# rvolden/C3POa

Measured on AMD Instinct MI355X. Metric: R2C2 reads->consensus/sec, higher is better.
Workload: dtype int32

## Files before the change

c3poa_amd/_lib.py:

```python
import ctypes as C
import os

import numpy as np

_HERE = os.path.dirname(os.path.abspath(__file__))
LIB_PATH = os.environ.get("C3POA_LIB", os.path.join(_HERE, "lib", "libc3poa_hip.so"))
MAX_PEAKS = 256

STAGE_CONK, STAGE_PEAKS, STAGE_POA, STAGE_POLISH, STAGES_ALL = 1, 2, 4, 8, 15
STAGE_QV = 16
QV_GLOBAL, QV_ANCHOR_START, QV_ANCHOR_END = 0, 1, 2
ST_OK, ST_NOT_ASSIGNED, ST_NO_PEAKS, ST_NO_CONSENSUS, ST_TOO_SHORT, ST_LIMIT = range(6)

EXPORTS = ["c3_default_config", "c3_version", "c3_device_count", "c3_warm_device", "c3_create", "c3_destroy", "c3_last_error", "c3_set_splints",
           "c3_batch_upload", "c3_batch_stage", "c3_batch_commit", "c3_batch_assign", "c3_batch_run", "c3_batch_sync", "c3_batch_results", "c3_batch_results_snapshot", "c3_batch_results_fetch", "c3_batch_timing",
           "c3_fetch_track", "c3_fetch_smoothed", "c3_fetch_raw_peaks", "c3_fetch_draft", "c3_fetch_msa2",
           "c3_call_peaks", "c3_poa_msa", "c3_pairwise_consensus", "c3_determine_consensus", "c3_zero_repeats", "c3_scan_splints",
           "c3_reader_open", "c3_reader_open_range", "c3_reader_close", "c3_reader_error", "c3_reader_names_only", "c3_reader_next", "c3_reader_next_set", "c3_reader_noqual", "c3_reader_reserved_bytes", "c3_reader_range_lost", "c3_write_group",
           "c3_scan_adapters", "c3_match_index", "c3_match_index_batch", "c3_demux_indexes", "c3_demux_host",
           "c3_assign_open", "c3_assign_close", "c3_assign_batch", "c3_assign_seen", "c3_write_splint_psl",
           "c3_host_alloc", "c3_host_free", "c3_writer_reset",
           "c3_batch_results_fetch_qv", "c3_batch_results_qv", "c3_batch_qv_timing", "c3_consensus_qv", "c3_consensus_qv_host",
           "c3_write_consensus_fastq",
           "c3_bgzf_create", "c3_bgzf_destroy", "c3_bgzf_bound", "c3_bgzf_compress", "c3_bgzf_compress_host",
           "c3_write_group_bgzf", "c3_write_consensus_fastq_bgzf",
           "c3_bgzf_scan", "c3_bgzf_decompress", "c3_bgzf_decompress_host", "c3_reader_open_inflate", "c3_reader_inflate_wait",
           "c3_fastq_parse", "c3_fastq_parse_host", "c3_reader_parse_on_device", "c3_reader_parse_stats", "c3_bam_parse", "c3_bam_parse_host",
           "c3_post_emit", "c3_post_emit_host", "c3_post_emit_timing",
           "c3_fasta_parse", "c3_fasta_parse_host", "c3_demux_emit", "c3_demux_emit_host", "c3_demux_emit_timing",
           "c3_emit_group", "c3_emit_group_host", "c3_batch_emit_snapshot", "c3_batch_emit_fetch", "c3_emit_timing_get", "c3_append_streams",
           "c3_fastx_strict_parse_host", "c3_post_emit_text", "c3_post_text_reset", "c3_post_text_timing_get",
           "c3_demux_emit_text", "c3_demux_emit_text_host", "c3_demux_text_reset", "c3_demux_text_timing_get",
           "c3_reader_stage_on_device", "c3_reader_device_group", "c3_reader_stage_stats"]


ZERO_MAX_CELLS = 16777216


class Config(C.Structure):
    _fields_ = ([("device", C.c_int), ("conk_match", C.c_int), ("conk_mismatch", C.c_int), ("conk_penalty", C.c_int),
                 ("sg_iters", C.c_int), ("sg_window", C.c_int), ("sg_order", C.c_int), ("mdistcutoff", C.c_int),
                 ("poa_match", C.c_int), ("poa_mismatch", C.c_int), ("poa_o1", C.c_int), ("poa_e1", C.c_int),
                 ("poa_o2", C.c_int), ("poa_e2", C.c_int), ("poa_band_b", C.c_int), ("poa_band_f", C.c_double),
                 ("pol_match", C.c_int), ("pol_mismatch", C.c_int), ("pol_gap", C.c_int), ("pol_window", C.c_int),
                 ("pol_q", C.c_int), ("dang_band", C.c_int), ("slots_poa", C.c_int), ("slots_win", C.c_int), ("zero", C.c_int),
                 ("zero_max_cells", C.c_int64)])


class ReadResult(C.Structure):
    _fields_ = [("status", C.c_int32), ("n_peaks", C.c_int32), ("n_sub", C.c_int32), ("has_front", C.c_int32),
                ("has_tail", C.c_int32), ("front_end", C.c_int32), ("tail_beg", C.c_int32), ("cons_len", C.c_int32),
                ("draft_len", C.c_int32), ("n_win", C.c_int32), ("peaks", C.c_int32 * MAX_PEAKS),
                ("sub_beg", C.c_int32 * MAX_PEAKS), ("sub_end", C.c_int32 * MAX_PEAKS)]


RESULT_DTYPE = np.dtype([("status", "<i4"), ("n_peaks", "<i4"), ("n_sub", "<i4"), ("has_front", "<i4"),
                         ("has_tail", "<i4"), ("front_end", "<i4"), ("tail_beg", "<i4"), ("cons_len", "<i4"),
                         ("draft_len", "<i4"), ("n_win", "<i4"), ("peaks", "<i4", (MAX_PEAKS,)),
                         ("sub_beg", "<i4", (MAX_PEAKS,)), ("sub_end", "<i4", (MAX_PEAKS,))])
assert RESULT_DTYPE.itemsize == C.sizeof(ReadResult)


class Timing(C.Structure):
    _fields_ = [(n, C.c_float) for n in ("ms_pack", "ms_conk", "ms_peaks", "ms_poa", "ms_prep", "ms_window",
                                         "ms_stitch", "ms_total")] + \
               [(n, C.c_int64) for n in ("n_reads", "n_bases", "n_windows", "cells_conk", "cells_poa", "cells_polish", "n_poa_redo")] + \
               [(n, C.c_float) for n in ("ms_wall", "ms_host_worklist", "ms_alloc", "ms_host_gap")] + \
               [(n, C.c_int64) for n in ("cells_polish_computed", "n_band_layers", "n_band_fallback", "n_band_mismatch", "n_win_redo", "n_poa_redo16")]


def _fields_dict(t):
    return {f[0]: getattr(t, f[0]) for f in t._fields_}


class _Info(C.Structure):

    def as_dict(self):
        return {k: int(getattr(self, k)) for k, _t in self._fields_}


class QvTiming(C.Structure):
    _fields_ = [("ms_qv", C.c_float)] + [(n, C.c_int64) for n in ("n_reads", "n_pieces", "n_skipped", "band_cells", "edge_hits")]


class FastaInfo(_Info):
    _fields_ = [(k, C.c_int64) for k in ("n_records", "consumed", "name_bytes", "base_bytes")] + [("departed", C.c_int32)]


class DemuxInfo(_Info):
    _fields_ = [(k, C.c_int64) for k in ("n_records", "n_kept", "consumed", "out_bytes")] + [("departed", C.c_int32)]


class DemuxTiming(C.Structure):
    _fields_ = [(n, C.c_float) for n in ("ms_parse", "ms_demux", "ms_emit", "ms_call")] + \
               [(n, C.c_int64) for n in ("n_records", "n_kept", "in_bytes", "out_bytes")]


class DemuxSetsStruct(C.Structure):
    _fields_ = [(k + f, t) for k in "ab" for f, t in (("_n", C.c_int), ("_cat", C.c_void_p), ("_off", C.c_void_p), ("_names", C.c_void_p), ("_name_off", C.c_void_p))]


class DemuxTextInfo(_Info):
    _fields_ = [(k, C.c_int64) for k in ("n_records", "n_kept", "consumed", "text_bytes", "out_bytes")] + \
               [(k, C.c_int32) for k in ("departed", "kind", "n_streams")]


class DemuxTextTiming(C.Structure):
    _fields_ = [(n, C.c_float) for n in ("ms_inflate", "ms_parse", "ms_demux", "ms_split", "ms_emit", "ms_bgzf", "ms_call")] + \
               [(n, C.c_int64) for n in ("n_records", "n_kept", "in_bytes", "text_bytes", "out_bytes")] + \
               [(n, C.c_int32) for n in ("n_streams", "n_waits")]


class FastqInfo(_Info):
    _fields_ = [(k, C.c_int64) for k in ("n_records", "n_kept", "n_short", "consumed", "name_bytes", "base_bytes")] + [("departed", C.c_int32)]


class BamInfo(_Info):
    _fields_ = [(k, C.c_int64) for k in ("n_records", "n_kept", "n_short", "consumed", "name_bytes", "base_bytes", "header_bytes", "bad_at")] + \
               [("departed", C.c_int32), ("reason", C.c_int32)]


class FastxInfo(_Info):
    _fields_ = [(k, C.c_int64) for k in ("n_records", "consumed", "name_bytes", "base_bytes")] + [("departed", C.c_int32)]


class PostTextInfo(_Info):
    _fields_ = [(k, C.c_int64) for k in ("n_records", "n_kept", "consumed", "text_bytes", "out_bytes")] + [("departed", C.c_int32)]


class PostTextTiming(C.Structure):
    _fields_ = [(n, C.c_float) for n in ("ms_inflate", "ms_parse", "ms_gather", "ms_adapter", "ms_post", "ms_bgzf", "ms_call")] + \
               [(n, C.c_int64) for n in ("n_records", "n_kept", "in_bytes", "text_bytes", "out_bytes")]


class PostArgs(C.Structure):
    _fields_ = [("n", C.c_int32), ("names", C.c_void_p), ("name_off", C.c_void_p), ("seqs", C.c_void_p), ("quals", C.c_void_p),
                ("off", C.c_void_p), ("table", C.c_void_p), ("n_ad", C.c_int32), ("ad_len", C.c_void_p), ("ad_class", C.c_void_p),
                ("class5", C.c_int32), ("ad_names", C.c_void_p), ("ad_name_off", C.c_void_p), ("has_index", C.c_int32),
                ("n_idx", C.c_int32), ("idx_cat", C.c_void_p), ("idx_off", C.c_void_p), ("idx_dest", C.c_void_p),
                ("n_dest", C.c_int32), ("undirectional", C.c_int32), ("trim", C.c_int32), ("barcoded", C.c_int32)]


class PostTiming(C.Structure):
    _fields_ = [(k, C.c_float) for k in ("ms_classify", "ms_scan", "ms_emit", "ms_call")] + \
               [(k, C.c_int64) for k in ("n_reads", "n_kept", "in_bytes", "out_bytes")]


class EmitTiming(C.Structure):
    _fields_ = [(k, C.c_float) for k in ("ms_len", "ms_scan", "ms_write", "ms_bgzf", "ms_call")] + \
               [(k, C.c_int64) for k in ("n_reads", "n_records", "in_bytes", "out_bytes")]


class HostBatchStruct(C.Structure):
    _fields_ = [("n", C.c_int32), ("n_short", C.c_int64), ("names", C.c_void_p), ("name_off", C.c_void_p),
                ("seqs", C.c_void_p), ("quals", C.c_void_p), ("off", C.c_void_p)]


class DeviceBatchStruct(C.Structure):
    _fields_ = [("d_seqs", C.c_void_p), ("d_quals", C.c_void_p), ("device", C.c_int32), ("bytes", C.c_int64)]


_lib = None


def load():
    global _lib
    if _lib is not None:
        return _lib
    if not os.path.exists(LIB_PATH):
        raise ImportError("c3poa_amd: %s is missing -- run `python -c 'import __graft_entry__ as g; g.build()'` "
                          "(there is no CPU fallback)" % LIB_PATH)
    lib = C.CDLL(LIB_PATH)
    vp, ip, cp, i64p = C.c_void_p, C.POINTER(C.c_int), C.c_char_p, C.c_void_p
    lib.c3_default_config.argtypes = [C.POINTER(Config)]
    lib.c3_version.restype = C.c_char_p
    lib.c3_create.argtypes = [C.POINTER(Config), C.POINTER(vp)]
    lib.c3_destroy.argtypes = [vp]
    lib.c3_destroy.restype = None
    lib.c3_last_error.argtypes = [vp]
    lib.c3_last_error.restype = C.c_char_p
    lib.c3_set_splints.argtypes = [vp, C.c_int, cp, i64p]
    lib.c3_batch_upload.argtypes = [vp, C.c_int, vp, vp, i64p, vp, vp]
    lib.c3_batch_stage.argtypes = [vp, C.c_int, vp, vp, i64p, vp, vp]
    lib.c3_batch_commit.argtypes = [vp]
    lib.c3_batch_assign.argtypes = [vp, vp, vp]
    lib.c3_batch_run.argtypes = [vp, C.c_int]
    lib.c3_batch_sync.argtypes = [vp]
    lib.c3_batch_results.argtypes = [vp, vp, vp, C.c_int64, i64p]
    lib.c3_batch_results_snapshot.argtypes = [vp]
    lib.c3_batch_results_fetch.argtypes = [vp, vp, vp, C.c_int64, i64p]
    lib.c3_batch_timing.argtypes = [vp, C.POINTER(Timing)]
    lib.c3_fetch_track.argtypes = [vp, C.c_int, vp, C.c_int64]
    lib.c3_fetch_smoothed.argtypes = [vp, C.c_int, vp, C.c_int64]
    lib.c3_fetch_raw_peaks.argtypes = [vp, C.c_int, vp, C.c_int]
    lib.c3_fetch_draft.argtypes = [vp, C.c_int, vp, C.c_int]
    lib.c3_fetch_msa2.argtypes = [vp, C.c_int, vp, vp, C.c_int]
    lib.c3_call_peaks.argtypes = [vp, vp, C.c_int, C.c_int, vp, C.c_int, vp]
    lib.c3_poa_msa.argtypes = [vp, C.c_int, C.POINTER(cp), ip, vp, C.c_int, ip, vp, C.c_int64, ip]
    lib.c3_zero_repeats.argtypes = [vp, cp, cp, C.c_int, cp, cp, C.c_int, C.c_int, vp, C.c_int, ip]
    lib.c3_scan_splints.argtypes = [vp, vp, vp, vp]
    lib.c3_pairwise_consensus.argtypes = [vp, cp, cp, C.c_int, cp, C.c_int, cp, cp, C.c_int, cp, vp, C.c_int, ip]
    lib.c3_scan_adapters.argtypes = [vp, vp]
    lib.c3_match_index.argtypes = [cp, C.c_int, C.c_int, cp, vp]
    lib.c3_match_index_batch.argtypes = [vp, C.c_int, vp, vp, C.c_int, cp, vp, vp]
    lib.c3_demux_indexes.argtypes = [vp, C.c_int, vp, C.c_int, cp, vp, C.c_int, cp, vp, vp, vp]
    lib.c3_demux_host.argtypes = [C.c_int, vp, C.c_int, cp, vp, C.c_int, cp, vp, vp, vp]
    lib.c3_assign_open.argtypes = [cp, C.c_int, C.POINTER(cp), C.POINTER(vp)]
    lib.c3_assign_close.argtypes = [vp]
    lib.c3_assign_close.restype = None
    lib.c3_assign_batch.argtypes = [vp, C.POINTER(HostBatchStruct), vp, vp]
    lib.c3_assign_seen.argtypes = [vp, vp, vp]
    lib.c3_write_splint_psl.argtypes = [C.POINTER(HostBatchStruct), vp, vp, vp, C.c_int, C.POINTER(cp), vp, C.c_int, cp, vp]
    lib.c3_host_alloc.argtypes = [C.c_int64, C.POINTER(vp)]
    lib.c3_host_free.argtypes = [vp]
    lib.c3_host_free.restype = None
    lib.c3_writer_reset.restype = None
    lib.c3_reader_open.argtypes = [cp, C.c_int, C.POINTER(vp)]
    lib.c3_reader_open_range.argtypes = [cp, C.c_int, C.c_int64, C.c_int64, C.POINTER(vp)]
    lib.c3_reader_close.argtypes = [vp]
    lib.c3_reader_close.restype = None
    lib.c3_reader_error.argtypes = [vp]
# ... 1464 lines not shown
```

c3poa_amd/csrc/c3_args.h:

```cpp
#pragma once
#include "c3_dev.h"
#include <cstddef>

struct C3Counters {
  int queue;
  int peaks_queue;
  unsigned long long cells;
  unsigned long long cells_computed;
  unsigned long long zero_cells;
  int poa_ovf;
  int poa_ovf16;
  int n_windows;
  int win_ovf;
  int win_queue2;
  int band_layers, band_fallback;
  int band_mismatch;
  struct { int window, layer, R, q, band_row, full_row, next_row; } verify;
  unsigned long long phases[16];
};
static_assert(offsetof(C3Counters, cells) % 8 == 0 && offsetof(C3Counters, cells_computed) % 8 == 0 &&
              offsetof(C3Counters, zero_cells) % 8 == 0 && offsetof(C3Counters, phases) % 8 == 0, "u64 counters must be 8-byte aligned");

struct ConkArgs {
  C3Batch b; const uint8_t* sp_codes; const int* sp_len; int32_t* track; C3Info* info; C3Counters* cnt;
  int match, mismatch, penalty;
  int n_spl; int32_t* scan;
};
struct PeaksArgs {
  C3Batch b; const int32_t* track; C3Info* info; double* bufA; double* bufB; int32_t* cand; uint8_t* cstate;
  int32_t* raw_peaks; int32_t* n_raw; const int* sp_len; double coef[64]; int64_t maxL; int window, iters, min_dist;
  C3Counters* cnt;
};
struct PoaArgs {
  C3Batch b; C3Info* info; C3Params p; C3Counters* cnt; const int* work; int n_work;
  int* ibase; int* ebase; char* cellsb; uint8_t* bbase; long long* score;
  int Ncap, K, Pcap, cells_cap;
  uint8_t* draft; int32_t* tpos; uint8_t* msa_dbg; const int64_t* msa_off; int* msa_len;
  int rb_span;
  int no2col;
  uint4* desc; int* jump;
  int* pbase;
  int* overflow;
  int* overflow16;
};
#define C3_POA_NI 19
__host__ __device__ inline int c3_poa_far_shift(bool w32) { return w32 ? 0 : 2; }
struct PoaLayout { size_t ints, edges, cells, bases, score, desc, jump, path, total; };
__host__ __device__ inline PoaLayout c3_poa_layout(size_t Ncap, size_t K, int cells_cap, int far_shift, size_t Pcap) {
  PoaLayout l;
  l.ints = sizeof(int) * C3_POA_NI * Ncap; l.edges = sizeof(int) * 3 * Ncap * K;
  l.cells = 2 * (size_t)cells_cap + 16 * (size_t)(cells_cap >> far_shift);
  l.bases = 5 * Ncap; l.score = sizeof(long long) * Ncap; l.desc = sizeof(uint4) * 2 * Ncap;
  l.jump = sizeof(int) * C3_JUMP_LEVELS * Ncap; l.path = sizeof(int) * Pcap;
  l.total = l.ints + l.edges + l.cells + l.bases + l.score + l.desc + l.jump + l.path;
  return l;
}

struct WLayer { int qbeg, len, begin, end; };
struct WinRec { int rid, w, n_layers, blen, tgs, out_len, polished, pad_; };
struct PrepArgs {
  C3Batch b; C3Info* info; C3Params p; C3Counters* cnt; const int* work; int n_work;
  const uint8_t* draft; int32_t* tpos; int wcap; uint8_t* eD; int64_t ecap; int* lw_first; int* lw_last; int NLcap, NWcap;
  WinRec* wrec; WLayer* wlay; int* win_base;
  int sub_shift;
  int rows_old;
};
struct WinArgs {
  C3Batch b; C3Params p; C3Counters* cnt; int n_win; const WinRec* wrec_in; WinRec* wrec; const WLayer* wlay; int NLcap;
  const uint8_t* draft;
  uint8_t* base; int* ibase; int* ebase; long long* score;
  int32_t* H; uint16_t* D; uint4* rdesc; int Ncap, K; long long hcap; uint8_t* wout; int wout_cap;
  int Lcap;
  int band_mode;
  const int* wlist; int* ovf_list;
  int no_chain;
};
#define W_INTS 19
struct WinLayout { size_t ints, edges, bases, score, H, D, desc, total; };
__host__ __device__ inline WinLayout c3_win_layout(size_t Ncap, size_t K, size_t hcap) {
  WinLayout l;
  l.ints = sizeof(int) * W_INTS * Ncap; l.edges = sizeof(int) * 4 * Ncap * K; l.bases = 2 * Ncap; l.score = sizeof(long long) * Ncap;
  l.H = sizeof(int32_t) * hcap; l.D = hcap; l.desc = sizeof(uint4) * (Ncap + 1);
  l.total = l.ints + l.edges + l.bases + l.score + l.H + l.D + l.desc;
  return l;
}
struct StitchArgs {
  C3Batch b; C3Info* info; const int* work; int n_work; const WinRec* wrec; const int* win_base; const uint8_t* wout; int wout_cap; char* cons;
  const uint8_t* zflag;
};
struct AdapterArgs {
  C3Batch b; C3Params p; C3Counters* cnt;
  const uint8_t* ad_codes; const int* ad_len; int n_ad;
  uint8_t* D; long long dcap;
  int32_t* out;
};

struct ZeroArgs {
  C3Batch b; C3Info* info; C3Params p; C3Counters* cnt; const int* work; int n_work;
  uint8_t* D; long long dcap;
  int4* zinfo; uint8_t* zflag;
  const uint8_t* draft; char* cons;
  uint8_t* S; long long scap; int zk;
};

struct ZlLayout { long long ck, dir, car, total; };
__host__ __device__ inline ZlLayout c3_zl_layout(long long n0, long long n1, long long K) {
  ZlLayout l;
  l.ck = 0;
  l.dir = (n1 + K - 1) / K * (n0 + 1) * 8;
  l.car = (l.dir + (n1 < K ? n1 : K) * (n0 + 1) + 15) & ~15LL;
  l.total = (l.car + n1 * 12 + 255) & ~255LL;
  return l;
}
struct QvArgs {
  int n_reads; const C3Info* info; const uint32_t* pk; const int64_t* woff; const uint8_t* qual; const int64_t* off;
  const char* cons; char* qv;
  int sa_np, sa_n; const int64_t* sa_woff; const int64_t* sa_off; const int32_t* sa_mode;
  uint32_t* dirs; long long dir_words;
  int* gS; uint8_t* gcodes; long long gcap;
  int lds_n;
  unsigned long long* cnt;
};
```

c3poa_amd/csrc/c3_handle.hip:

```cpp
#include "c3_host.h"
#include "c3_bgzf.h"

thread_local double c3h::g_alloc_ms = 0.0;

__device__ __forceinline__ uint32_t pack_code(uint32_t b) {
  const uint32_t u = b & 0xDFu;
  const uint32_t c = (u >> 1) & 3u;
  const bool ok = (u == 'A') | (u == 'C') | (u == 'G') | (u == 'T') | (u == 'U');
  return ok ? (c ^ (c >> 1)) : 0u;
}
__global__ __launch_bounds__(256) void k_pack(const uint8_t* ascii, const int64_t* off, const int64_t* woff, int n, uint32_t* pk) {
  const int lane = threadIdx.x & 63;
  const int wave = (blockIdx.x * blockDim.x + threadIdx.x) >> 6, n_waves = (gridDim.x * blockDim.x) >> 6;
  for (int r = wave; r < n; r += n_waves) {
    const int64_t L = off[r + 1] - off[r];
    const int64_t nw = woff[r + 1] - woff[r];
    const uint8_t* s = ascii + off[r];
    uint32_t* dst = pk + woff[r];
    for (int64_t w = lane; w < nw; w += 64) {
      uint32_t x = 0;
      if (w * 16 + 16 <= L) {
        uint32_t v[4];
        __builtin_memcpy(v, s + w * 16, 16);
#pragma unroll
// ... 20 lines not shown
__device__ __forceinline__ long long cons_len_of(const C3Info* p) { return p->status == C3_ST_OK ? (long long)p->cons_len : 0; }
__global__ __launch_bounds__(256) void k_coff_sums(const C3Info* info, int n, long long* part) {
  __shared__ long long sh[256];
  const int i = blockIdx.x * 256 + threadIdx.x;
  sh[threadIdx.x] = i < n ? cons_len_of(info + i) : 0;
  __syncthreads();
  for (int d = 128; d > 0; d >>= 1) { if ((int)threadIdx.x < d) sh[threadIdx.x] += sh[threadIdx.x + d]; __syncthreads(); }
  if (threadIdx.x == 0) part[blockIdx.x] = sh[0];
}
__global__ __launch_bounds__(1024) void k_coff_scan(long long* part, int nb, int64_t* coff, int n) {
  __shared__ long long sh[1024];
  long long carry = 0;
  for (int b0 = 0; b0 < nb; b0 += 1024) {
    const int b = b0 + threadIdx.x;
    const long long v = b < nb ? part[b] : 0;
    sh[threadIdx.x] = v;
    __syncthreads();
    for (int d = 1; d < 1024; d <<= 1) { long long t = (int)threadIdx.x >= d ? sh[threadIdx.x - d] : 0; __syncthreads(); sh[threadIdx.x] += t; __syncthreads(); }
    if (b < nb) part[b] = carry + sh[threadIdx.x] - v;
    carry += sh[1023];
    __syncthreads();
  }
  if (threadIdx.x == 0) { coff[0] = 0; coff[n] = carry; }
}
__global__ __launch_bounds__(256) void k_coff_final(const C3Info* info, int n, const long long* part, int64_t* coff) {
  __shared__ long long sh[256];
  const int i = blockIdx.x * 256 + threadIdx.x;
  sh[threadIdx.x] = i < n ? cons_len_of(info + i) : 0;
  __syncthreads();
  for (int d = 1; d < 256; d <<= 1) { long long t = (int)threadIdx.x >= d ? sh[threadIdx.x - d] : 0; __syncthreads(); sh[threadIdx.x] += t; __syncthreads(); }
  if (i < n) coff[i + 1] = part[blockIdx.x] + sh[threadIdx.x];
}
__global__ void k_init_info(C3Info* info, int n) {
  int i = blockIdx.x * blockDim.x + threadIdx.x;
  if (i < n) { C3Info* p = &info[i]; p->status = C3_ST_OK; p->n_peaks = 0; p->n_sub = 0; p->has_front = p->has_tail = 0;
               p->front_end = p->tail_beg = 0; p->cons_len = 0; p->draft_len = 0; p->n_win = 0; }
}

extern "C" void c3_default_config(c3_config* c) {
  memset(c, 0, sizeof(*c));
  c->device = 0;
  c->conk_match = 5; c->conk_mismatch = -4; c->conk_penalty = 20;
  c->sg_iters = 3; c->sg_window = 41; c->sg_order = 2; c->mdistcutoff = 500;
  c->poa_match = 5; c->poa_mismatch = 4; c->poa_o1 = 4; c->poa_e1 = 2; c->poa_o2 = 24; c->poa_e2 = 1;
  c->poa_band_b = 10; c->poa_band_f = 0.01;
  c->pol_match = 3; c->pol_mismatch = -5; c->pol_gap = -4; c->pol_window = 500; c->pol_q = 5; c->dang_band = 128;
  c->slots_poa = 0; c->slots_win = 0; c->zero = 1; c->zero_max_cells = 16 << 20;
}
extern "C" const char* c3_version(void) { return "c3poa_amd 0.1 (gfx950)"; }
extern "C" int c3_device_count(void) { int n = 0; if (hipGetDeviceCount(&n) != hipSuccess) { (void)hipGetLastError(); return 0; } return n; }

extern "C" int c3_warm_device(int device) {
  int n = 0;
  if (hipGetDeviceCount(&n) != hipSuccess || device < 0 || device >= n) { (void)hipGetLastError(); return C3_E_NO_DEVICE; }
  if (hipSetDevice(device) != hipSuccess || hipFree(nullptr) != hipSuccess) { (void)hipGetLastError(); return C3_E_HIP; }
  return C3_E_OK;
}

static thread_local std::string g_create_err;
extern "C" const char* c3_last_error(const c3_handle* h) { return h ? h->err.c_str() : g_create_err.c_str(); }
void c3_set_host_error(const char* msg) { g_create_err = msg; }

static int check_poa_scoring(const c3_config* cfg) {
  const struct { const char* name; int v, lo, hi; } f[6] = {
    {"poa_match", cfg->poa_match, 1, 64}, {"poa_mismatch", cfg->poa_mismatch, 0, 64},
    {"poa_o1", cfg->poa_o1, 0, 64}, {"poa_e1", cfg->poa_e1, 0, 16}, {"poa_o2", cfg->poa_o2, 0, 64}, {"poa_e2", cfg->poa_e2, 0, 16}};
  for (const auto& x : f) {
    if (x.v < x.lo || x.v > x.hi) {
      char buf[160];
      snprintf(buf, sizeof buf, "%s = %d: must be %d..%d (the 16-bit cells of k_poa and their guard are exact in that range only)", x.name, x.v, x.lo, x.hi);
      return host_fail(C3_E_ARG, buf);
    }
  }
  return C3_E_OK;
}

static int check_pol_scoring(const c3_config* cfg) {
  const struct { const char* name; int v; } f[3] = {{"pol_match", cfg->pol_match}, {"pol_mismatch", cfg->pol_mismatch}, {"pol_gap", cfg->pol_gap}};
  for (const auto& x : f) {
    if (x.v < -C3_POL_MAX || x.v > C3_POL_MAX) {
      char buf[160];
      snprintf(buf, sizeof buf, "%s = %d: must be %d..%d (the 32-bit cells of the polish rows and their sentinels are exact in that range only)", x.name, x.v, -C3_POL_MAX, C3_POL_MAX);
      return host_fail(C3_E_ARG, buf);
    }
  }
  if (cfg->pol_match <= 2 * cfg->pol_gap) {
    char buf[200];
    snprintf(buf, sizeof buf, "pol_match = %d: must be above 2 * pol_gap = %d (a match that scores no more than two gaps makes every layer a chain of new nodes, beyond the window graph's capacity)",
             cfg->pol_match, 2 * cfg->pol_gap);
    return host_fail(C3_E_ARG, buf);
  }
  return C3_E_OK;
}

static int check_pol_window(const c3_config* cfg) {
  char buf[200];
  if (cfg->pol_window < 1 || cfg->pol_window > C3_POL_WINDOW_MAX) {
    snprintf(buf, sizeof buf, "pol_window = %d: must be %d..%d (a window graph of 3 * pol_window + 40 nodes per layer has to stay below the 65535 node ids k_window's consensus holds)",
             cfg->pol_window, 1, C3_POL_WINDOW_MAX);
    return host_fail(C3_E_ARG, buf);
  }
  if (cfg->dang_band < 0) {
    snprintf(buf, sizeof buf, "dang_band = %d: must be %d..%d (the half width of the extension band; 0 is the diagonal alone)", cfg->dang_band, 0, 255);
    return host_fail(C3_E_ARG, buf);
  }
  return C3_E_OK;
}

extern "C" int c3_create(const c3_config* cfg, c3_handle** out) {
  if (!cfg || !out) return C3_E_ARG;
  *out = nullptr;
  if (int rc = check_poa_scoring(cfg)) return rc;
  if (int rc = check_pol_scoring(cfg)) return rc;
  if (int rc = check_pol_window(cfg)) return rc;
  int ndev = 0;
  hipError_t e = hipGetDeviceCount(&ndev);
  if (e != hipSuccess || ndev <= 0) return host_fail(C3_E_NO_DEVICE, "no HIP device: the c3poa HIP backend has no CPU fallback");
  if (cfg->device < 0 || cfg->device >= ndev) return host_fail(C3_E_ARG, "bad device ordinal");
  if (cfg->conk_match < -127 || cfg->conk_match > 127 || cfg->conk_mismatch < -127 || cfg->conk_mismatch > 127) {
    return host_fail(C3_E_ARG, "conk_match / conk_mismatch must fit a signed byte");
  }
  if (cfg->dang_band > 255) return host_fail(C3_E_LIMIT, "dang_band must be at most 255 (k_prep holds 512 band offsets per wave)");
  if (cfg->sg_order != 2 && cfg->sg_order != 3) return host_fail(C3_E_ARG, "sg_order must be 2 or 3");
  if (cfg->sg_window < 5 || cfg->sg_window > 127 || !(cfg->sg_window & 1)) return host_fail(C3_E_ARG, "sg_window must be odd, 5..127");
  if (cfg->zero_max_cells < 1 || cfg->zero_max_cells > INT32_MAX) return host_fail(C3_E_ARG, "zero_max_cells must be 1..2147483647");
  c3_handle* h = new c3_handle();
  h->cfg = *cfg;
  hipDeviceProp_t prop;
  e = hipSetDevice(cfg->device);
  if (e == hipSuccess) {
    (void)hipSetDeviceFlags(hipDeviceScheduleBlockingSync); (void)hipGetLastError();
    e = hipGetDeviceProperties(&prop, cfg->device);
  }
  if (e == hipSuccess) e = hipStreamCreate(&h->stream);
  if (e == hipSuccess) e = hipStreamCreate(&h->stream_up);
  if (e == hipSuccess) e = hipStreamCreate(&h->stream_dn);
  if (e == hipSuccess) e = hipEventCreateWithFlags(&h->ev_dn, hipEventDisableTiming);
  if (e == hipSuccess) e = hipHostMalloc((void**)&h->h_tot, 64, hipHostMallocDefault);
  for (int i = 0; i < 2 && e == hipSuccess; ++i) e = hipEventCreate(&h->ev_up[i]);
  for (int i = 0; i < EV_N && e == hipSuccess; ++i) e = hipEventCreate(&h->ev[i]);
  if (e != hipSuccess) { c3_destroy(h); return host_fail(C3_E_HIP, hipGetErrorString(e)); }
  h->n_cus = prop.multiProcessorCount > 0 ? prop.multiProcessorCount : 256;
  h->mem_total = prop.totalGlobalMem;
  memset(&h->tm, 0, sizeof(h->tm));
  *out = h;
  return C3_E_OK;
}

extern "C" void c3_destroy(c3_handle* h) {
  if (!h) return;
  (void)hipSetDevice(h->cfg.device);
  for (hipStream_t s : {h->stream, h->stream_up, h->stream_dn}) if (s) (void)hipStreamSynchronize(s);
  for (hipStream_t s : {h->stream, h->stream_up, h->stream_dn}) if (s) (void)hipStreamDestroy(s);
  for (hipEvent_t ev : {h->ev_dn, h->ev_up[0], h->ev_up[1], h->ev_qv[0], h->ev_qv[1]}) if (ev) (void)hipEventDestroy(ev);
  for (hipEvent_t ev : h->ev) if (ev) (void)hipEventDestroy(ev);
  for (hipEvent_t ev : h->ev_post) if (ev) (void)hipEventDestroy(ev);
  for (hipEvent_t ev : h->ev_fa) if (ev) (void)hipEventDestroy(ev);
  for (c3h::EmitBufs* eb : {&h->emit_sa, &h->emit_snap}) for (hipEvent_t ev : eb->ev) if (ev) (void)hipEventDestroy(ev);
  if (h->ev_emit_dn) (void)hipEventDestroy(h->ev_emit_dn);
  if (h->h_fa_hdr) (void)hipHostFree(h->h_fa_hdr);
  c3h::post_text_free(h);
  c3h::demux_text_free(h);
  if (h->h_tot) (void)hipHostFree(h->h_tot);
  delete h;
}

extern "C" int c3_set_splints(c3_handle* h, int n, const char* cat, const int64_t* off) {
  if (!h || n <= 0 || !cat || !off) return C3_E_ARG;
  HIPCHK(hipSetDevice(h->cfg.device));
  std::vector<uint8_t> codes((size_t)n * 2 * C3_SPLINT_MAX, 0);
  std::vector<int> sp_len((size_t)n, 0); int max_spl = 0;
  for (int i = 0; i < n; ++i) {
    int S = (int)(off[i + 1] - off[i]);
    if (S <= 0 || S > C3_SPLINT_MAX) return c3_fail(h, C3_E_LIMIT, "splint length must be 1..512");
    if ((long long)std::max({h->cfg.conk_match, h->cfg.conk_mismatch, 0}) * S > 32000 || h->cfg.conk_penalty < 0 || h->cfg.conk_penalty > 32000)
      return c3_fail(h, C3_E_LIMIT, "max(conk_match, conk_mismatch) * splint length and conk_penalty must stay within 32000 (16-bit score cells in k_conk)");
    sp_len[(size_t)i] = S; max_spl = std::max(max_spl, S);
    for (int k = 0; k < S; ++k) {
      int c = code_of(cat[off[i] + k]);
      codes[((size_t)i * 2 + 0) * C3_SPLINT_MAX + k] = (uint8_t)c;
      codes[((size_t)i * 2 + 1) * C3_SPLINT_MAX + (S - 1 - k)] = (uint8_t)(3 - c);
    }
  }
  HIPCHK(h->d_sp_codes.put(codes.data(), codes.size(), h->stream));
  HIPCHK(h->d_sp_len.put(sp_len.data(), sizeof(int) * n, h->stream));
  HIPCHK(hipStreamSynchronize(h->stream));
  h->sp_len.swap(sp_len); h->max_spl = max_spl; h->n_spl = n;
  return C3_E_OK;
}

extern "C" int c3_batch_stage(c3_handle* h, int n, const char* seqs, const char* quals, const int64_t* off,
                              const int16_t* splint_id, const char* strand) {
  if (!h || n <= 0 || !seqs || !quals || !off || !strand) return C3_E_ARG;
  if (h->n_spl <= 0) return c3_fail(h, C3_E_STATE, "c3_set_splints must be called first");
  if (h->st.pending) return c3_fail(h, C3_E_STATE, "a staged batch is waiting for c3_batch_commit");
  HIPCHK(hipSetDevice(h->cfg.device));
  if (off[0] != 0) return c3_fail(h, C3_E_ARG, "off[0] must be 0");
  c3_handle::Staged& t = h->st;
  t.n = n; t.total = off[n] - off[0]; t.off.assign(off, off + n + 1); t.woff.assign(n + 1, 0); t.maxL = 0;
  t.sid.assign((size_t)n, 0); t.strand.assign(strand, (size_t)n);
  for (int i = 0; i < n; ++i) {
    int64_t L = off[i + 1] - off[i];
    if (L < 0 || L > (1 << 30)) return c3_fail(h, C3_E_ARG, "bad read length");
    t.maxL = std::max(t.maxL, L);
    t.woff[i + 1] = t.woff[i] + (L + 15) / 16 + 2;
    if (splint_id) { if (splint_id[i] < 0 || splint_id[i] >= h->n_spl) return c3_fail(h, C3_E_ARG, "splint_id out of range"); t.sid[i] = splint_id[i]; }
  }
  t.words = t.woff[n];
  const size_t T = (size_t)t.total;
  HIPCHK(t.d_ascii.ensure(T + 16)); HIPCHK(t.d_pk.ensure(sizeof(uint32_t) * (size_t)t.words + 64));
  HIPCHK(t.d_qual.ensure(T + 16)); HIPCHK(t.d_off.ensure(sizeof(int64_t) * (n + 1))); HIPCHK(t.d_woff.ensure(sizeof(int64_t) * (n + 1)));
  HIPCHK(t.d_strand.ensure(n)); HIPCHK(t.d_sid.ensure(sizeof(int16_t) * n));
  hipStream_t su = h->stream_up;
  HIPCHK(hipEventRecord(h->ev_up[0], su));
  HIPCHK(hipMemcpyAsync(t.d_ascii.p, seqs, T, hipMemcpyHostToDevice, su));
  HIPCHK(hipMemcpyAsync(t.d_qual.p, quals, T, hipMemcpyHostToDevice, su));
  HIPCHK(hipMemcpyAsync(t.d_off.p, t.off.data(), sizeof(int64_t) * (n + 1), hipMemcpyHostToDevice, su));
  HIPCHK(hipMemcpyAsync(t.d_woff.p, t.woff.data(), sizeof(int64_t) * (n + 1), hipMemcpyHostToDevice, su));
  HIPCHK(hipMemcpyAsync(t.d_strand.p, t.strand.data(), n, hipMemcpyHostToDevice, su));
  HIPCHK(hipMemcpyAsync(t.d_sid.p, t.sid.data(), sizeof(int16_t) * n, hipMemcpyHostToDevice, su));
  c3k_launch_pack(t.d_ascii.as<uint8_t>(), t.d_off.as<int64_t>(), t.d_woff.as<int64_t>(), n, t.d_pk.as<uint32_t>(), std::min((n + 3) / 4, h->n_cus * 32), su);
  HIPCHK(hipEventRecord(h->ev_up[1], su));
  HIPCHK(hipGetLastError());
  t.pending = true;
  return C3_E_OK;
}

extern "C" int c3_batch_commit(c3_handle* h) {
  if (!h) return C3_E_ARG;
  if (!h->st.pending) return c3_fail(h, C3_E_STATE, "no staged batch");
  HIPCHK(hipSetDevice(h->cfg.device));
  HIPCHK(hipStreamSynchronize(h->stream));
  HIPCHK(hipStreamSynchronize(h->stream_up));
  c3_handle::Staged& t = h->st;
  std::swap(h->d_ascii, t.d_ascii); std::swap(h->d_pk, t.d_pk); std::swap(h->d_woff, t.d_woff); std::swap(h->d_qual, t.d_qual);
  std::swap(h->d_off, t.d_off); std::swap(h->d_strand, t.d_strand); std::swap(h->d_sid, t.d_sid);
  h->off.swap(t.off); h->woff.swap(t.woff);
  h->n = t.n; h->total = t.total; h->words = t.words; h->maxL = t.maxL;
  t.pending = false;
  const int n = h->n;
  HIPCHK(h->d_info.ensure(sizeof(C3Info) * (size_t)n));
  HIPCHK(h->d_counter.ensure(sizeof(C3Counters)));
  HIPCHK(hipMemsetAsync(h->d_info.p, 0, sizeof(C3Info) * (size_t)n, h->stream));
  hipLaunchKernelGGL(k_init_info, dim3((n + 255) / 256), dim3(256), 0, h->stream, h->d_info.as<C3Info>(), n);
  HIPCHK(hipStreamSynchronize(h->stream));
  HIPCHK(hipGetLastError());
  float ms = 0; HIPCHK(hipEventElapsedTime(&ms, h->ev_up[0], h->ev_up[1]));
  memset(&h->tm, 0, sizeof(h->tm)); h->tm.ms_pack = ms; h->tm.n_reads = n; h->tm.n_bases = h->total;
  h->stages_done = 0; h->injected = false; h->n_windows = 0; h->res_prefix = 0;
  return C3_E_OK;
}

extern "C" int c3_batch_assign(c3_handle* h, const int16_t* splint_id, const char* strand) {
  if (!h || h->n <= 0 || !splint_id || !strand) return C3_E_ARG;
  HIPCHK(hipSetDevice(h->cfg.device));
  std::vector<int16_t> sid((size_t)h->n);
  for (int i = 0; i < h->n; ++i) {
    const bool on = strand[i] == '+' || strand[i] == '-';
    if (on && (splint_id[i] < 0 || splint_id[i] >= h->n_spl)) return c3_fail(h, C3_E_ARG, "splint_id out of range");
    sid[(size_t)i] = on ? splint_id[i] : (int16_t)0;
  }
  HIPCHK(hipMemcpyAsync(h->d_strand.p, strand, (size_t)h->n, hipMemcpyHostToDevice, h->stream));
  HIPCHK(hipMemcpyAsync(h->d_sid.p, sid.data(), sizeof(int16_t) * (size_t)h->n, hipMemcpyHostToDevice, h->stream));
  hipLaunchKernelGGL(k_init_info, dim3((h->n + 255) / 256), dim3(256), 0, h->stream, h->d_info.as<C3Info>(), h->n);
  HIPCHK(hipStreamSynchronize(h->stream));
  HIPCHK(hipGetLastError());
  h->stages_done = 0;
  return C3_E_OK;
}

extern "C" int c3_batch_upload(c3_handle* h, int n, const char* seqs, const char* quals, const int64_t* off,
                               const int16_t* splint_id, const char* strand) {
  if (h && h->st.pending) { (void)hipStreamSynchronize(h->stream_up); h->st.pending = false; }
  int rc = c3_batch_stage(h, n, seqs, quals, off, splint_id, strand);
  if (rc != C3_E_OK) return rc;
  return c3_batch_commit(h);
}

extern "C" int c3_batch_qv_timing(c3_handle* h, c3_qv_timing* t) {
  if (!h || !t) return C3_E_ARG;
  *t = h->qtm;
  return C3_E_OK;
}

extern "C" int c3_batch_sync(c3_handle* h) {
  if (!h) return C3_E_ARG;
  HIPCHK(hipSetDevice(h->cfg.device));
  HIPCHK(hipStreamSynchronize(h->stream));
  return C3_E_OK;
}

extern "C" int c3_batch_results_snapshot(c3_handle* h) {
  if (!h || h->n <= 0) return C3_E_ARG;
  if (h->snap_pending.load(std::memory_order_acquire)) return c3_fail(h, C3_E_STATE, "c3_batch_results_snapshot: the previous snapshot has not been fetched");
  HIPCHK(hipSetDevice(h->cfg.device));
  const int n = h->n;
  DBuf& d_coff = h->d_gather_off; DBuf& d_out = h->d_gather;
  const int nb = (n + 255) / 256;
  HIPCHK(d_coff.ensure(sizeof(int64_t) * (size_t)(n + 1))); HIPCHK(h->d_coff_part.ensure(sizeof(long long) * (size_t)nb));
  hipLaunchKernelGGL(k_coff_sums, dim3(nb), dim3(256), 0, h->stream, h->d_info.as<C3Info>(), n, h->d_coff_part.as<long long>());
  hipLaunchKernelGGL(k_coff_scan, dim3(1), dim3(1024), 0, h->stream, h->d_coff_part.as<long long>(), nb, d_coff.as<int64_t>(), n);
  hipLaunchKernelGGL(k_coff_final, dim3(nb), dim3(256), 0, h->stream, h->d_info.as<C3Info>(), n, h->d_coff_part.as<long long>(), d_coff.as<int64_t>());
  long long tot = 0;
  const bool have_cons = (h->stages_done & C3_STAGE_POLISH) != 0;
  if (have_cons) {
    HIPCHK(hipMemcpyAsync(h->h_tot, d_coff.as<int64_t>() + n, sizeof(long long), hipMemcpyDeviceToHost, h->stream));
    HIPCHK(hipStreamSynchronize(h->stream));
// ... 269 lines not shown
```

c3poa_amd/csrc/c3_host.h:

```cpp
#pragma once
#include "c3_dev.h"
#include "c3_args.h"
#include "c3_launch.h"
#include "c3_checks.h"
#include "c3_emit.h"
#include "c3_post.h"
#include "c3_fastx.h"
#include "c3_dsplit.h"
#include "c3_bgzf.h"
#include <algorithm>
#include <atomic>
#include <chrono>
#include <cstddef>
#include <cstdio>
#include <cstdlib>
#include <cstring>
#include <functional>
#include <string>
#include <vector>

struct c3_handle;
namespace c3h {
extern thread_local double g_alloc_ms;
int qv_scratch(c3_handle* h, long long max_m, long long max_n, int n_items, QvArgs& a, int* grid);
int fetch_msa_rows(c3_handle* h, int read, int nrows, char* out, int64_t cap, int* msa_len);
struct EmitBufs;
int emit_run(c3_handle* h, EmitArgs& p, EmitBufs& eb, hipStream_t s, std::vector<int64_t>& so, int64_t cap);
int post_sizes(c3_handle* h, const c3_post_args* a, PostArgs& p, std::vector<int64_t>& so);
int post_write(c3_handle* h, PostArgs& p, int64_t need);
int adapters_device(c3_handle* h, const C3Batch& b, int64_t max_len, int32_t* d_out);
int bgzf_inflate_to_device(c3_bgzf* z, const char* src, int64_t n, int64_t nm, uint8_t* d_dst, int64_t* out_len);
namespace fa { enum { FA_TEXT, FA_CNT, FA_NL, FA_LSE, FA_LDST, FA_BSUM, FA_HDR, FA_OFF, FA_NOFF, FA_RECL, FA_HASH, FA_NAMES, FA_SEQS, FA_KREC, FA_ROFF,
                      FA_OUT, FA_ANAMES, FA_ANO, FA_BNAMES, FA_BNO, FA_N }; }
int fasta_parse_resident(c3_handle* h, const uint8_t* d_text, int64_t n, int at_eof, int kept, FaArgs* a);
int fasta_gather_resident(c3_handle* h, FaArgs* a);
int demux_sets_device(c3_handle* h, const c3_demux_sets* st, const uint8_t* tab, int K, int64_t nk, FaArgs* a);
struct ZStage;
struct ZStatus { hipError_t e = hipSuccess; enum { OK, MEMBER_SIZE, BEYOND_BOUND } bad = OK; const char* what = ""; int waits = 0; };
typedef std::function<hipError_t(char* d_zin, int64_t c0, int64_t cn)> ZStageIn;
ZStatus bgzf_chunks(ZStage& z, hipStream_t s, int64_t len, const ZStageIn& stage_in, char* arena, int64_t cap, int64_t* out, bool wait_after_copy_out);
struct TextFront;
struct TextLoad { int nxt = 0, kind = 0, waits = 0; int64_t total = 0; float ms_inflate = 0; };
void text_free(TextFront& t);
void text_reset(TextFront& t);
int text_load(c3_handle* h, TextFront& t, const char* src, int64_t n, bool in_z, bool keep_q, const char* who, const char* keep_flag,
              hipEvent_t* ev, int n_ev, TextLoad* ld);
int text_tables(c3_handle* h, TextFront& t, const TextLoad& ld, int at_eof, FxArgs& f, int* waits, hipEvent_t ev_begin = nullptr, hipEvent_t ev_records = nullptr);
int text_gather(c3_handle* h, TextFront& t, FxArgs& f, bool keep_q, hipEvent_t ev_begin = nullptr);
void text_commit(TextFront& t, const TextLoad& ld, int64_t consumed, int at_eof);
int bgzf_stream_device(c3_handle* h, ZStage& z, const char* d_src, int64_t len, char* arena, int64_t cap, int64_t* out, int* waits = nullptr);
void post_text_free(c3_handle* h);
void demux_text_free(c3_handle* h);
}

#define BGZF_CHUNK_BLOCKS 2048

static inline double dbg_now_ms() { using namespace std::chrono; return duration<double, std::milli>(steady_clock::now().time_since_epoch()).count(); }
#define DBG(...) do { if (getenv("C3_DEBUG")) { fprintf(stderr, "[c3 %.3f] ", dbg_now_ms()); fprintf(stderr, __VA_ARGS__); fflush(stderr); } } while (0)

struct DBuf {
  void* p = nullptr; size_t cap = 0;
  DBuf() = default;
  DBuf(DBuf&& o) noexcept : p(o.p), cap(o.cap) { o.p = nullptr; o.cap = 0; }
  DBuf& operator=(DBuf&& o) noexcept { std::swap(p, o.p); std::swap(cap, o.cap); return *this; }
  DBuf(const DBuf&) = delete;
  DBuf& operator=(const DBuf&) = delete;
  ~DBuf() { if (p) (void)hipFree(p); }
  hipError_t ensure(size_t bytes) {
    if (bytes <= cap) return hipSuccess;
    const double t0 = dbg_now_ms();
    if (p) { hipError_t e = hipFree(p); p = nullptr; cap = 0; if (e != hipSuccess) return e; }
    size_t want = bytes + bytes / 8 + 256;
    hipError_t e = hipMalloc(&p, want);
    if (e == hipSuccess) cap = want;
    if (e == hipSuccess && getenv("C3_DEBUG_POISON")) e = hipMemset(p, 0xA5, want);
    c3h::g_alloc_ms += dbg_now_ms() - t0;
    return e;
  }
  hipError_t put(const void* src, size_t bytes, hipStream_t s, size_t slack = 0) {
    const hipError_t e = ensure(bytes + slack);
    return e != hipSuccess ? e : hipMemcpyAsync(p, src, bytes, hipMemcpyHostToDevice, s);
  }
  template <class T> T* as() const { return (T*)p; }
};

struct c3h::EmitBufs { DBuf work, offs, arena; hipEvent_t ev[5] = {}; };

struct c3h::ZStage {
  DBuf zin, zslots, zsizes, zpacked; int* h_sizes = nullptr;
  ~ZStage() { if (h_sizes) (void)hipHostFree(h_sizes); }
  hipError_t pin() { return h_sizes ? hipSuccess : hipHostMalloc((void**)&h_sizes, BGZF_CHUNK_BLOCKS * sizeof(int), hipHostMallocDefault); }
  hipError_t reserve(int64_t cn) {
    cn = std::min(cn, (int64_t)BGZF_CHUNK_BLOCKS * BGZF_BLOCK);
    const size_t nb = (size_t)((cn + BGZF_BLOCK - 1) / BGZF_BLOCK);
    hipError_t e = pin();
    if (e == hipSuccess) e = zin.ensure((size_t)cn + 256);
    if (e == hipSuccess) e = zslots.ensure(nb * BGZF_SLOT);
    if (e == hipSuccess) e = zsizes.ensure(nb * sizeof(int));
    if (e == hipSuccess) e = zpacked.ensure(nb * BGZF_MAX_MEMBER);
    return e;
  }
};
struct c3h::TextFront {
  DBuf text[2]; int cur = 0, kind = 0; int64_t text_n = 0, tail_from = 0;
  DBuf cnt, nl, slen, nlen, bsum, hdr, lhdr, off, name_off, woff, src, hash, names, seqs, quals;
  ZStage zs;
  C3FxHdr* h_hdr = nullptr; C3FqHdr* h_lhdr = nullptr; c3_bgzf* z = nullptr;
};
struct PostText : c3h::TextFront {
  DBuf pk, table;
  hipEvent_t ev[8] = {};
  c3_post_text_timing tm = {};
};
struct DemuxText : c3h::TextFront {
  DBuf krec, kb, nkept, key, rank, base, soff, out;
  int64_t* h_soff = nullptr;
  hipEvent_t ev[6] = {};
  c3_demux_text_timing tm = {};
};

struct Summary { int status, n_sub, max_sub, sum_sub, max_dang, front, tail, n_peaks; };
enum { EV_N = 10 };
struct c3_handle {
  c3_config cfg; std::string err; hipStream_t stream = nullptr; int n_cus = 256; size_t mem_total = 0;
  hipStream_t stream_up = nullptr; hipEvent_t ev_up[2] = {nullptr, nullptr};
  hipStream_t stream_dn = nullptr; hipEvent_t ev_dn = nullptr; long long* h_tot = nullptr;
  std::atomic<bool> snap_pending{false}; int snap_n = 0, snap_kp = 0; long long snap_tot = 0; bool snap_cons = false;
  DBuf d_info_snap, d_coff_part;
  struct Staged { DBuf d_ascii, d_pk, d_woff, d_qual, d_off, d_strand, d_sid; std::vector<int64_t> off, woff; std::vector<int16_t> sid; std::string strand;
                  int n = 0; int64_t total = 0, words = 0, maxL = 0; bool pending = false; } st;
  hipEvent_t ev[EV_N] = {};
  int n_spl = 0, max_spl = 0; std::vector<int> sp_len; DBuf d_sp_codes, d_sp_len;
  int n = 0; int64_t total = 0, words = 0, maxL = 0; std::vector<int64_t> off, woff;
  DBuf d_ascii, d_pk, d_woff, d_qual, d_off, d_strand, d_sid, d_info, d_track, d_draft, d_tpos, d_cons, d_counter, d_gather, d_gather_off;
  DBuf d_raw, d_nraw, d_sum, d_work, d_bufA, d_bufB, d_cand, d_cst, d_msa, d_msa_off, d_msa_len;
  DBuf s_poa_i, s_poa_nk, s_poa_cells, s_poa_b, s_poa_sc, s_poa_desc, s_poa_jump, s_poa_path, d_overflow;
  int n_poa_redo = 0;
  int n_poa_redo16 = 0;
  DBuf s_eD, s_lw, d_wrec, d_wlay, d_wbase, d_wout;
  DBuf s_win_i, s_win_nk, s_win_h, s_win_d, s_win_b, s_win_sc, s_win_desc, s_win_h2, s_win_d2, d_wovf;
  DBuf s_zero_d, d_zinfo, d_zflag, d_zwork; std::vector<int> zwork;
  DBuf s_zero_l;
  DBuf d_dmx_heads, d_dmx_meta, d_dmx_out;
  DBuf d_qv, s_qv_dirs, s_qv_g, d_qv_cnt, d_gather_qv;
  hipEvent_t ev_qv[2] = {nullptr, nullptr}; c3_qv_timing qtm = {}; bool snap_qv = false;
  DBuf d_post[16]; hipEvent_t ev_post[5] = {}; c3_post_timing ptm = {};
  PostText pt;
  DemuxText dx; std::vector<uint32_t> dmx_meta_host;
  DBuf d_fa[20]; hipEvent_t ev_fa[10] = {}; c3_demux_timing dtm = {}; struct C3FaHdr* h_fa_hdr = nullptr;
  DBuf d_emit[10]; c3h::EmitBufs emit_sa; c3_emit_timing etm = {};
  c3h::EmitBufs emit_snap; DBuf d_emit_names, d_emit_noff; c3h::ZStage emit_zs;
  hipEvent_t ev_emit_dn = nullptr;
  std::atomic<bool> emit_pending{false}; int emit_S = 0, emit_flags = 0; std::vector<int64_t> emit_so; c3_emit_timing emit_tm = {};
  std::vector<Summary> sum; std::vector<int> work;
  int res_prefix = 0;
  int peaks_grid = 0; bool debug_msa = false; bool injected = false;
  int n_windows = 0;
  c3_timing tm;
  unsigned long long phase_poa[16] = {0}, phase_win[16] = {0};
  int stages_done = 0;
};

static inline int c3_hip_fail(c3_handle* h, hipError_t e, const char* what, const char* file, int line) {
  char buf[512];
  const char* base = strrchr(file, '/');
  snprintf(buf, sizeof buf, "HIP error %d (%s) at %s:%d: %s", (int)e, hipGetErrorString(e), base ? base + 1 : file, line, what);
  if (h) h->err = buf;
  return C3_E_HIP;
}
static inline int c3_fail(c3_handle* h, int code, const char* msg) { if (h) h->err = msg; return code; }
#define HIPCHK(x) do { hipError_t e_ = (x); if (e_ != hipSuccess) return c3_hip_fail(h, e_, #x, __FILE__, __LINE__); } while (0)
static inline int host_fail(int code, const char* msg) { c3_set_host_error(msg); return code; }
static inline int bgzf_fail(hipError_t e, const char* what) {
  char buf[256];
  snprintf(buf, sizeof buf, "HIP error %d (%s): %s", (int)e, hipGetErrorString(e), what);
  return host_fail(C3_E_HIP, buf);
}
#define ZCHK(x, what) do { hipError_t e_ = (x); if (e_ != hipSuccess) return bgzf_fail(e_, what); } while (0)

template <class T> struct Override {
  T& ref; const T saved;
  Override(T& r, T v) : ref(r), saved(r) { r = v; }
  ~Override() { ref = saved; }
  Override(const Override&) = delete;
};

static inline C3Counters* dev_cnt(c3_handle* h) { return h->d_counter.as<C3Counters>(); }
template <class T> static inline hipError_t zero_cnt(c3_handle* h, T* field) { return hipMemsetAsync(field, 0, sizeof(T), h->stream); }
static inline hipError_t read_counters(c3_handle* h, C3Counters* c) {
  hipError_t e = hipMemcpyAsync(c, h->d_counter.p, sizeof(*c), hipMemcpyDeviceToHost, h->stream);
  return e != hipSuccess ? e : hipStreamSynchronize(h->stream);
}

static inline int code_of(char c) {
  switch (c) { case 'C': case 'c': return 1; case 'G': case 'g': return 2; case 'T': case 't': case 'U': case 'u': return 3; default: return 0; }
}

static inline C3Batch dev_batch(c3_handle* h) {
  C3Batch b; b.n = h->n; b.pk = h->d_pk.as<uint32_t>(); b.woff = h->d_woff.as<int64_t>(); b.qual = h->d_qual.as<uint8_t>();
  b.off = h->d_off.as<int64_t>(); b.strand = h->d_strand.as<uint8_t>(); b.splint_id = h->d_sid.as<int16_t>();
  return b;
}
static inline C3Params dev_params(const c3_config& c) {
  C3Params p;
  p.conk_match = c.conk_match; p.conk_mismatch = c.conk_mismatch; p.conk_penalty = c.conk_penalty;
  p.sg_iters = c.sg_iters; p.sg_window = c.sg_window; p.sg_order = c.sg_order; p.mdist = c.mdistcutoff;
  p.poa_match = c.poa_match; p.poa_mismatch = c.poa_mismatch; p.o1 = c.poa_o1; p.e1 = c.poa_e1; p.o2 = c.poa_o2; p.e2 = c.poa_e2;
  p.band_b = c.poa_band_b; p.band_f = c.poa_band_f;
  p.pol_match = c.pol_match; p.pol_mismatch = c.pol_mismatch; p.pol_gap = c.pol_gap; p.pol_window = c.pol_window; p.pol_q = c.pol_q;
  p.dang_band = c.dang_band;
  p.zero = c.zero; p.zr_match = 2; p.zr_mismatch = 4; p.zr_gapo = 4; p.zr_gape = 2; p.zr_min_score = 80; p.zr_max_cells = (int)c.zero_max_cells;
  return p;
}

struct c3_bgzf {
  int device = 0; hipStream_t stream = nullptr;
  c3h::ZStage zs;
  C3BgzfMember* h_mem = nullptr; int2* h_res = nullptr;
  DBuf d_mem, d_res, d_out;
  struct FqSlot {
    DBuf text, names, seqs, quals, off, name_off, src;
    int64_t text_n = 0, n_rec = 0;
    int64_t* h_off = nullptr; int64_t* h_name_off = nullptr; size_t h_cap = 0;
  } fq[2];
  DBuf d_cnt, d_nl, d_slen, d_nlen, d_bsum, d_hdr;
  C3FqHdr* h_hdr = nullptr;
  DBuf d_tiles, d_rpos, d_reason, d_rsrc, d_bhdr;
  C3BamHdr* h_bhdr = nullptr;
  hipStream_t copy_stream = nullptr;
  struct DevSet { DBuf seqs, quals; };
  std::vector<DevSet> dsets;
};
```

c3poa_amd/csrc/c3_launch.h:

```cpp
#pragma once
#include <hip/hip_runtime.h>
#include <stddef.h>
#include <stdint.h>

struct ConkArgs; struct AdapterArgs; struct PostArgs; struct PeaksArgs; struct PoaArgs; struct PrepArgs; struct WinArgs; struct StitchArgs;
struct ZeroArgs; struct QvArgs; struct C3BgzfMember; struct C3FqHdr; struct C3BamHdr; struct C3BamTile; struct FaArgs; struct EmitArgs; struct FxArgs; struct DsArgs;

extern "C" {
void c3k_launch_conk(const ConkArgs*, int, int, int, hipStream_t);
void c3k_launch_adapter(const AdapterArgs*, int, hipStream_t);
void c3k_launch_match_index(const char*, const int*, int, int, const char*, const long long*, int*, hipStream_t);
void c3k_launch_pairwise(const uint8_t*, int, const uint8_t*, int, const uint8_t*, int, uint8_t*, uint8_t*, int*, hipStream_t);
void c3k_launch_poa(const PoaArgs*, int, int, int, hipStream_t);
void c3k_launch_post_classify(const PostArgs*, hipStream_t);
void c3k_launch_post_scan(const PostArgs*, hipStream_t);
void c3k_launch_post_emit(const PostArgs*, hipStream_t);
void c3k_launch_demux(const uint8_t*, int, const uint8_t*, int, int, int, int32_t*, uint8_t*, hipStream_t);
size_t c3k_demux_lds(int, int);
void c3k_launch_peaks(const PeaksArgs*, int, hipStream_t);
int c3k_peaks_blocks_per_cu(void);
void c3k_launch_prep(const PrepArgs*, int, hipStream_t);
void c3k_launch_window(const WinArgs*, int, hipStream_t);
void c3k_launch_stitch(const StitchArgs*, int, hipStream_t);
void c3k_launch_zero(const ZeroArgs*, int, hipStream_t);
void c3k_launch_zero_long(const ZeroArgs*, int, hipStream_t);
void c3k_launch_zero_finish(const ZeroArgs*, int, hipStream_t);
void c3k_launch_qv(const QvArgs*, int, hipStream_t);
int c3k_qv_lds_max(void);
void c3k_launch_bgzf(const uint8_t*, long long, int, uint8_t*, int*, uint8_t*, hipStream_t);
void c3k_launch_inflate(const uint8_t*, const C3BgzfMember*, int, uint8_t*, int2*, hipStream_t);
void c3k_launch_fastq_count(const uint8_t*, uint32_t, uint32_t, int32_t*, int, C3FqHdr*, hipStream_t);
void c3k_launch_fastq_lines(const uint8_t*, uint32_t, uint32_t, const int32_t*, int32_t*, hipStream_t);
void c3k_launch_fastq_records(const uint8_t*, uint32_t, uint32_t, const int32_t*, int, int, int, int, int32_t*, int32_t*, long long*,
                              C3FqHdr*, int64_t*, int64_t*, int4*, hipStream_t);
void c3k_launch_fastq_gather(const uint8_t*, const int4*, const int64_t*, const int64_t*, long long, uint8_t*, uint8_t*, uint8_t*, hipStream_t);
void c3k_launch_bam_chain(const uint8_t*, uint32_t, uint32_t, int, C3BamTile*, C3BamHdr*, hipStream_t);
void c3k_launch_bam_records(const uint8_t*, uint32_t, uint32_t, const C3BamTile*, int, int, int, uint32_t*, int32_t*, int32_t*, int32_t*,
                            int4*, long long*, C3BamHdr*, int64_t*, int64_t*, int4*, hipStream_t);
void c3k_launch_bam_gather(const uint8_t*, const int4*, const int64_t*, const int64_t*, long long, uint8_t*, uint8_t*, uint8_t*, hipStream_t);
void c3k_launch_fasta_count(const FaArgs*, hipStream_t);
void c3k_launch_fasta_records(const FaArgs*, int, hipStream_t);
void c3k_launch_fasta_gather(const FaArgs*, hipStream_t);
void c3k_launch_demux_heads(const FaArgs*, hipStream_t);
void c3k_launch_demux_len(const FaArgs*, hipStream_t);
void c3k_launch_demux_emit(const FaArgs*, hipStream_t);
void c3k_launch_emit_len(const EmitArgs*, hipStream_t);
void c3k_launch_emit_scan(const EmitArgs*, hipStream_t);
void c3k_launch_emit_write(const EmitArgs*, hipStream_t);
void c3k_launch_fastx_high(const FxArgs*, hipStream_t);
void c3k_launch_fastx_records(const FxArgs*, hipStream_t);
void c3k_launch_fastx_gather(const FxArgs*, hipStream_t);
void c3k_launch_dsplit_krec(const DsArgs*, hipStream_t);
void c3k_launch_dsplit_place(const DsArgs*, hipStream_t);
void c3k_launch_dsplit_emit(const DsArgs*, hipStream_t);
void c3k_launch_pack(const uint8_t*, const int64_t*, const int64_t*, int, uint32_t*, int, hipStream_t);
}
```

c3poa_amd/csrc/c3_stages.hip:

```cpp
#include "c3_host.h"

__global__ void k_summary(const C3Info* info, const int64_t* off, int n, Summary* out) {
  int i = blockIdx.x * blockDim.x + threadIdx.x;
  if (i >= n) return;
  const C3Info* p = &info[i];
  Summary s; s.status = p->status; s.n_sub = p->n_sub; s.max_sub = 0; s.sum_sub = 0; s.max_dang = 0; s.n_peaks = p->n_peaks;
  for (int k = 0; k < p->n_sub; ++k) { int l = p->sub_end[k] - p->sub_beg[k]; s.sum_sub += l; if (l > s.max_sub) s.max_sub = l; }
  int L = (int)(off[i + 1] - off[i]);
  s.front = p->has_front ? p->front_end : 0; s.tail = p->has_tail ? L - p->tail_beg : 0;
  if (p->has_front) s.max_dang = p->front_end;
  if (p->has_tail && L - p->tail_beg > s.max_dang) s.max_dang = L - p->tail_beg;
  out[i] = s;
}

static hipError_t zero_counters(c3_handle* h) { return hipMemsetAsync(h->d_counter.p, 0, sizeof(C3Counters), h->stream); }

static int auto_slots(c3_handle* h, int want, size_t per_slot_bytes, int n_items, int waves_per_cu) {
  int s = want > 0 ? want : h->n_cus * waves_per_cu;
  size_t budget = h->mem_total ? h->mem_total / 3 : ((size_t)64 << 30);
  if (per_slot_bytes > 0) { size_t mx = budget / per_slot_bytes; if ((size_t)s > mx) s = (int)std::max<size_t>(mx, 1); }
  if (s > n_items) s = std::max(n_items, 1);
  return s;
}

// ... 6 lines not shown
  int waves = std::min(h->n, h->n_cus * 32);
  c3k_launch_conk(&a, h->max_spl, (waves + 3) / 4, 0, h->stream);
  HIPCHK(hipGetLastError());
  return 0;
}

static void savgol_coeffs(int window, double* c) {
  int m = (window - 1) / 2;
  double den = (double)(2 * m - 1) * (double)(2 * m + 1) * (double)(2 * m + 3);
  for (int k = -m; k <= 0; ++k) c[k + m] = 3.0 * (double)(3 * m * m + 3 * m - 1 - 5 * k * k) / den;
}

static int run_peaks(c3_handle* h) {
  static const int blocks_per_cu = c3k_peaks_blocks_per_cu();
  const int grid = std::min(h->n, h->n_cus * blocks_per_cu);
  h->peaks_grid = grid;
  const size_t mL = (size_t)h->maxL + 8;
  HIPCHK(h->d_bufA.ensure(sizeof(double) * mL * grid)); HIPCHK(h->d_bufB.ensure(sizeof(double) * mL * grid));
  HIPCHK(h->d_cand.ensure(sizeof(int32_t) * (mL / 2 + 2) * grid)); HIPCHK(h->d_cst.ensure((mL / 2 + 2) * grid));
  HIPCHK(h->d_raw.ensure(sizeof(int32_t) * (size_t)h->n * C3_MAX_PEAKS)); HIPCHK(h->d_nraw.ensure(sizeof(int32_t) * (size_t)h->n));
  PeaksArgs a; memset(&a, 0, sizeof(a));
  a.b = dev_batch(h); a.track = h->d_track.as<int32_t>(); a.info = h->d_info.as<C3Info>();
  a.bufA = h->d_bufA.as<double>(); a.bufB = h->d_bufB.as<double>(); a.cand = h->d_cand.as<int32_t>(); a.cstate = h->d_cst.as<uint8_t>();
  a.raw_peaks = h->d_raw.as<int32_t>(); a.n_raw = h->d_nraw.as<int32_t>(); a.sp_len = h->d_sp_len.as<int>();
  savgol_coeffs(h->cfg.sg_window, a.coef);
  a.maxL = (int64_t)mL; a.window = h->cfg.sg_window; a.iters = h->cfg.sg_iters; a.min_dist = h->cfg.mdistcutoff;
  a.cnt = dev_cnt(h);
  HIPCHK(zero_cnt(h, &a.cnt->peaks_queue));
  c3k_launch_peaks(&a, grid, h->stream);
  HIPCHK(hipGetLastError());
  return 0;
}

static int copy_summary(c3_handle* h) {
  const int n = h->n;
  HIPCHK(h->d_sum.ensure(sizeof(Summary) * (size_t)n));
  hipLaunchKernelGGL(k_summary, dim3((n + 255) / 256), dim3(256), 0, h->stream, h->d_info.as<C3Info>(), h->d_off.as<int64_t>(), n, h->d_sum.as<Summary>());
  h->sum.resize(n);
  HIPCHK(hipMemcpyAsync(h->sum.data(), h->d_sum.p, sizeof(Summary) * (size_t)n, hipMemcpyDeviceToHost, h->stream));
  if (!getenv("C3_NO_SPIN")) {
    hipError_t q;
    while ((q = hipStreamQuery(h->stream)) == hipErrorNotReady) { for (int k_ = 0; k_ < 64; ++k_) __builtin_ia32_pause(); }
    if (q != hipSuccess) HIPCHK(q);
  }
  HIPCHK(hipStreamSynchronize(h->stream));
  int k = 2;
  for (int i = 0; i < n; ++i) k = std::max(k, std::max(h->sum[i].n_peaks, h->sum[i].n_sub));
  h->res_prefix = std::min((k + 7) & ~7, (int)C3_MAX_PEAKS);
  return 0;
}

static void fill_zero_args(c3_handle* h, ZeroArgs& z, int nz) {
  memset(&z, 0, sizeof(z));
  z.b = dev_batch(h); z.info = h->d_info.as<C3Info>(); z.p = dev_params(h->cfg); z.cnt = dev_cnt(h);
  z.work = h->d_zwork.as<int>(); z.n_work = nz;
  z.D = h->s_zero_d.as<uint8_t>(); z.zinfo = h->d_zinfo.as<int4>(); z.zflag = h->d_zflag.as<uint8_t>();
  z.draft = h->d_draft.as<uint8_t>(); z.cons = h->d_cons.as<char>();
}

static const long long ZL_BUDGET = 1LL << 30;
static int run_zero(c3_handle* h) {
  h->zwork.clear();
  HIPCHK(h->d_zflag.ensure((size_t)h->n + 16));
  HIPCHK(hipMemsetAsync(h->d_zflag.p, 0, (size_t)h->n, h->stream));
  if (!h->cfg.zero || h->injected) return 0;
  const char* ev_long = getenv("C3_DEBUG_ZERO_LONG");
  const bool force_long = ev_long && atoi(ev_long) != 0;
  const char* ev_k = getenv("C3_DEBUG_ZERO_K");
  const int zk = (ev_k && atoi(ev_k) > 0) ? atoi(ev_k) : 256;
  long long dmax = 0, smax = 0;
  std::vector<int> zlong;
  for (int i = 0; i < h->n; ++i) {
    const Summary& s = h->sum[i];
    if (s.status != C3_ST_NO_CONSENSUS || s.n_sub != 0 || s.front <= 0 || s.tail <= 0) continue;
    const long long cells = (long long)s.front * s.tail;
    if (cells > h->cfg.zero_max_cells) continue;
    if (!force_long && s.front <= 4096 && cells <= (16 << 20)) {
      h->zwork.push_back(i);
      dmax = std::max(dmax, (long long)(s.front + 1) * (s.tail + 1));
    } else {
      zlong.push_back(i);
      smax = std::max(smax, c3_zl_layout(s.front, s.tail, zk).total);
    }
  }
  const int ns = (int)h->zwork.size(), nl = (int)zlong.size();
  h->zwork.insert(h->zwork.end(), zlong.begin(), zlong.end());
  const int nz = ns + nl;
  if (nz == 0) return 0;
  HIPCHK(h->d_zwork.ensure(sizeof(int) * (size_t)nz)); HIPCHK(h->d_zinfo.ensure(sizeof(int4) * (size_t)h->n));
  if (ns) {
    const int grid = std::min(ns, 512);
    HIPCHK(h->s_zero_d.ensure((size_t)dmax * grid + 64));
  }
  int grid_l = 0;
  if (nl) {
    grid_l = (int)std::min<long long>(std::min(nl, 2 * h->n_cus), std::max(1LL, ZL_BUDGET / smax));
    HIPCHK(h->s_zero_l.ensure((size_t)smax * grid_l));
  }
  HIPCHK(hipMemcpyAsync(h->d_zwork.p, h->zwork.data(), sizeof(int) * (size_t)nz, hipMemcpyHostToDevice, h->stream));
  if (ns) {
    ZeroArgs z; fill_zero_args(h, z, ns); z.dcap = dmax;
    DBG("zero: nz=%d grid=%d dmax=%lld\n", ns, std::min(ns, 512), dmax);
    c3k_launch_zero(&z, std::min(ns, 512), h->stream);
    HIPCHK(hipGetLastError());
  }
  if (nl) {
    ZeroArgs z; fill_zero_args(h, z, nl);
    z.work = h->d_zwork.as<int>() + ns; z.S = h->s_zero_l.as<uint8_t>(); z.scap = smax; z.zk = zk;
    DBG("zero long: nz=%d grid=%d slot=%lld K=%d\n", nl, grid_l, smax, zk);
    c3k_launch_zero_long(&z, grid_l, h->stream);
    HIPCHK(hipGetLastError());
  }
  { int r_ = copy_summary(h); DBG("zero done\n"); return r_; }
}

static int fetch_summary(c3_handle* h) {
  int rc = copy_summary(h);
  DBG("summary copied\n");
  if (rc) return rc;
  const auto wl0 = std::chrono::steady_clock::now();
  struct WlTimer { c3_handle* h; std::chrono::steady_clock::time_point t0; ~WlTimer() { h->tm.ms_host_worklist = std::chrono::duration<float, std::milli>(std::chrono::steady_clock::now() - t0).count(); } } wl_timer_{h, wl0};
  HIPCHK(zero_cnt(h, &dev_cnt(h)->zero_cells));
  if ((rc = run_zero(h))) return rc;
  const int n = h->n;
  h->work.clear();
  for (int i = 0; i < n; ++i) if (h->sum[i].status == C3_ST_OK && h->sum[i].n_sub >= 1) h->work.push_back(i);
  if (n < (1 << 24)) {
    const size_t m = h->work.size();
    std::vector<uint64_t> keys(m), tmp(m);
    for (size_t k = 0; k < m; ++k) {
      const int i = h->work[k];
      const uint64_t cost = (uint64_t)h->sum[i].sum_sub * (uint64_t)h->sum[i].n_sub;
      keys[k] = ((((uint64_t)1 << 40) - 1 - cost) << 24) | (uint64_t)i;
    }
    uint64_t* src = keys.data(); uint64_t* dst = tmp.data();
    for (int pass = 0; pass < 4; ++pass) {
      const int sh = 24 + 10 * pass;
      size_t cnt[1025] = {0};
      for (size_t k = 0; k < m; ++k) ++cnt[((src[k] >> sh) & 1023) + 1];
      for (int b = 0; b < 1024; ++b) cnt[b + 1] += cnt[b];
      for (size_t k = 0; k < m; ++k) dst[cnt[(src[k] >> sh) & 1023]++] = src[k];
      std::swap(src, dst);
    }
    for (size_t k = 0; k < m; ++k) h->work[k] = (int)(src[k] & 0xffffff);
  } else {
    std::stable_sort(h->work.begin(), h->work.end(), [&](int x, int y) {
      long cx = (long)h->sum[x].sum_sub * h->sum[x].n_sub, cy = (long)h->sum[y].sum_sub * h->sum[y].n_sub; return cx > cy; });
  }
  HIPCHK(h->d_work.ensure(sizeof(int) * std::max<size_t>(h->work.size(), 1)));
  if (!h->work.empty()) HIPCHK(hipMemcpyAsync(h->d_work.p, h->work.data(), sizeof(int) * h->work.size(), hipMemcpyHostToDevice, h->stream));
  return 0;
}

static int launch_poa(c3_handle* h, const int* d_work, int nw, int Ncap, int K, int Pcap, long long cells, int* d_overflow, int* d_overflow16, int waves_per_cu, int wide_ring) {
  cells = (cells + 15) & ~15LL;
  cells = (cells + 63) & ~63LL;
  const bool w32 = d_overflow16 == nullptr || getenv("C3_DEBUG_POA32");
  const PoaLayout L = c3_poa_layout(Ncap, K, (int)cells, c3_poa_far_shift(w32), Pcap);
  const int slots = auto_slots(h, h->cfg.slots_poa, L.total, nw, waves_per_cu);
  const size_t S = (size_t)slots;
  HIPCHK(h->s_poa_i.ensure(L.ints * S)); HIPCHK(h->s_poa_nk.ensure(L.edges * S));
  HIPCHK(h->s_poa_cells.ensure(L.cells * S + 256)); HIPCHK(h->s_poa_b.ensure(L.bases * S)); HIPCHK(h->s_poa_sc.ensure(L.score * S));
  HIPCHK(h->s_poa_desc.ensure(L.desc * S)); HIPCHK(h->s_poa_jump.ensure(L.jump * S)); HIPCHK(h->s_poa_path.ensure(L.path * S));
  PoaArgs a; memset(&a, 0, sizeof(a));
  a.b = dev_batch(h); a.info = h->d_info.as<C3Info>(); a.p = dev_params(h->cfg);
  a.cnt = dev_cnt(h); a.work = d_work; a.n_work = nw;
  a.ibase = h->s_poa_i.as<int>(); a.ebase = h->s_poa_nk.as<int>(); a.cellsb = h->s_poa_cells.as<char>();
  a.bbase = h->s_poa_b.as<uint8_t>(); a.score = h->s_poa_sc.as<long long>();
  a.Ncap = Ncap; a.K = K; a.Pcap = Pcap; a.cells_cap = (int)cells; a.desc = h->s_poa_desc.as<uint4>(); a.jump = h->s_poa_jump.as<int>();
  a.pbase = h->s_poa_path.as<int>(); a.overflow = d_overflow; a.overflow16 = d_overflow16;
  if (const char* e = getenv("C3_DEBUG_POA_RBSPAN")) a.rb_span = std::max(3300, atoi(e));
  a.no2col = getenv("C3_DEBUG_POA_NO2COL") != nullptr;
  a.draft = h->d_draft.as<uint8_t>(); a.tpos = h->d_tpos.as<int32_t>();
  a.msa_dbg = nullptr; a.msa_off = nullptr; a.msa_len = nullptr;
  if (h->debug_msa) { a.msa_dbg = h->d_msa.as<uint8_t>(); a.msa_off = h->d_msa_off.as<int64_t>(); a.msa_len = h->d_msa_len.as<int>(); }
  DBG("poa: nw=%d Ncap=%d K=%d cells=%lld slots=%d (%.1f MB per slot)%s\n", nw, Ncap, K, cells, slots, L.total / 1048576.0, d_overflow ? "" : (d_overflow16 ? " [full-size pass]" : " [32-bit pass]"));
  c3k_launch_poa(&a, slots, w32 ? 1 : 0, wide_ring, h->stream);
  HIPCHK(hipGetLastError());
  return 0;
}

static int run_poa(c3_handle* h) {
  const int nw = (int)h->work.size();
  HIPCHK(h->d_draft.ensure((size_t)h->total + 64)); HIPCHK(h->d_tpos.ensure(sizeof(int32_t) * (size_t)h->total + 64));
  HIPCHK(h->d_cons.ensure((size_t)h->total + 64));
  HIPCHK(hipMemsetAsync(h->d_tpos.p, 0xff, sizeof(int32_t) * (size_t)h->total, h->stream));
  if (nw == 0) return 0;
  int max_sum = 0, max_ns = 0, max_q = 0;
  for (int i : h->work) { max_sum = std::max(max_sum, h->sum[i].sum_sub); max_ns = std::max(max_ns, h->sum[i].n_sub); max_q = std::max(max_q, h->sum[i].max_sub); }
  const int Ncap_full = max_sum + 8, K = max_ns + 1, Pcap = max_sum + 8;
  const int w = h->cfg.poa_band_b + (int)(h->cfg.poa_band_f * max_q);
  long long cells_full = (long long)(2 * max_q + 2) * (2 * w + 1 + max_q / 5);
  if (max_ns < 2) cells_full = 64;
  if (cells_full > 0x7fffff00LL) cells_full = 0x7fffff00LL;
  const double nodes_typ = (double)max_q * (1.0 + 0.15 * std::max(0, max_ns - 1));
  int Ncap = (int)std::min<double>(Ncap_full, 1.3 * nodes_typ + 256);
  long long cells = std::min<long long>(cells_full, (long long)(1.5 * nodes_typ * (2 * w + 12)) + 4096);
  if (const char* e_ = getenv("C3_DEBUG_POA_SMALL")) { Ncap = std::min(Ncap_full, std::max(64, atoi(e_))); cells = std::min<long long>(cells_full, 16LL * Ncap); }
  if (h->debug_msa) {
    std::vector<int64_t> mo(h->n + 1, 0);
    for (int i = 0; i < h->n; ++i) mo[i + 1] = mo[i] + (int64_t)h->sum[i].n_sub * (h->sum[i].sum_sub + 2);
    HIPCHK(h->d_msa.ensure((size_t)mo[h->n] + 64)); HIPCHK(h->d_msa_off.ensure(sizeof(int64_t) * (h->n + 1))); HIPCHK(h->d_msa_len.ensure(sizeof(int) * h->n));
    HIPCHK(hipMemcpyAsync(h->d_msa_off.p, mo.data(), sizeof(int64_t) * (h->n + 1), hipMemcpyHostToDevice, h->stream));
    HIPCHK(hipMemsetAsync(h->d_msa_len.p, 0, sizeof(int) * h->n, h->stream));
    HIPCHK(hipStreamSynchronize(h->stream));
  }
  HIPCHK(h->d_overflow.ensure(sizeof(int) * 2 * (size_t)nw));
  C3Counters* dc = dev_cnt(h);
  HIPCHK(zero_cnt(h, &dc->queue)); HIPCHK(zero_cnt(h, &dc->cells)); HIPCHK(zero_cnt(h, &dc->poa_ovf)); HIPCHK(zero_cnt(h, &dc->poa_ovf16));
  HIPCHK(zero_cnt(h, &dc->phases));
  int wide_ring = (max_q > 1792 || 2 * w + 1 + 24 > 128) ? 1 : 0;
  if (const char* e_ = getenv("C3_DEBUG_POA_WIDE")) wide_ring = atoi(e_) ? 1 : 0;
  int* ovA = h->d_overflow.as<int>(); int* ovB = h->d_overflow.as<int>() + nw;
  int rc = launch_poa(h, h->d_work.as<int>(), nw, Ncap, K, Pcap, cells, ovA, ovB, 24, wide_ring);
  if (rc) return rc;
  h->n_poa_redo = 0; h->n_poa_redo16 = 0;
  C3Counters c;
  HIPCHK(read_counters(h, &c));
  if (c.poa_ovf > 0) {
    h->n_poa_redo = c.poa_ovf;
    HIPCHK(zero_cnt(h, &dc->queue));
    if ((rc = launch_poa(h, ovA, c.poa_ovf, Ncap_full, K, Pcap, cells_full, nullptr, ovB, 24, wide_ring))) return rc;
    HIPCHK(read_counters(h, &c));
  }
  if (c.poa_ovf16 > 0) {
    h->n_poa_redo += c.poa_ovf16; h->n_poa_redo16 = c.poa_ovf16;
    HIPCHK(zero_cnt(h, &dc->queue));
    if ((rc = launch_poa(h, ovB, c.poa_ovf16, Ncap_full, K, Pcap, cells_full, nullptr, nullptr, 24, 0))) return rc;
  }
  if (!h->zwork.empty()) {
    ZeroArgs z; fill_zero_args(h, z, (int)h->zwork.size());
    c3k_launch_zero_finish(&z, std::min((int)h->zwork.size(), 512), h->stream);
    HIPCHK(hipGetLastError());
  }
  HIPCHK(hipMemcpyAsync(h->phase_poa, dc->phases, sizeof(h->phase_poa), hipMemcpyDeviceToHost, h->stream));
  return 0;
}

static int run_polish(c3_handle* h, float* ms_prep, float* ms_win, float* ms_st) {
  const int nw = (int)h->work.size();
  DBG("polish: nw=%d\n", nw);
  HIPCHK(h->d_cons.ensure((size_t)h->total + 64));
  if (nw == 0) return 0;
  const int WL = h->cfg.pol_window;
  int max_ns = 0, max_q = 0, max_dang = 0; long long wcap = 0;
  for (int i : h->work) {
    max_ns = std::max(max_ns, h->sum[i].n_sub); max_q = std::max(max_q, h->sum[i].max_sub); max_dang = std::max(max_dang, h->sum[i].max_dang);
    wcap += (2 * h->sum[i].max_sub + WL - 1) / WL + 1;
  }
  {
    const int pm = std::max({std::abs(h->cfg.pol_match), std::abs(h->cfg.pol_mismatch), std::abs(h->cfg.pol_gap)});
    const long long kstep = 4LL * pm + 3, bw = 2LL * h->cfg.dang_band + 1;
    if (kstep * (2LL * std::max(max_q, max_dang) + 4 * bw) >= C3_POL_KEY_RANGE)
      return c3_fail(h, C3_E_LIMIT, "polish scoring times the longest subread or dangling piece of the batch leaves the 32-bit cells of the polish rows: "
                                    "(4 * max|pol_*| + 3) * (2 * length + 4 * (2 * dang_band + 1)) must stay below 2^28");
  }
  const int NLcap = max_ns + 2, NWcap = (2 * max_q + WL - 1) / WL + 1;
  const int64_t ecap = (int64_t)(max_dang / (2 * h->cfg.dang_band + 1 > 320 ? 2 : 3) + 2) * 256;
  const size_t per_slot_prep = (size_t)ecap + (size_t)NLcap * NWcap * 8;
  const int slots_p = auto_slots(h, h->cfg.slots_poa, per_slot_prep, nw, getenv("C3_DEBUG_PREP_WPC") ? atoi(getenv("C3_DEBUG_PREP_WPC")) : 20);
  HIPCHK(h->s_eD.ensure((size_t)ecap * slots_p));
  HIPCHK(h->s_lw.ensure(sizeof(int) * (size_t)NLcap * NWcap * 2 * slots_p));
  HIPCHK(h->d_wrec.ensure(sizeof(WinRec) * (size_t)wcap)); HIPCHK(h->d_wlay.ensure(sizeof(WLayer) * (size_t)wcap * NLcap));
  HIPCHK(h->d_wbase.ensure(sizeof(int) * (size_t)h->n));
  PrepArgs p; memset(&p, 0, sizeof(p));
  p.b = dev_batch(h); p.info = h->d_info.as<C3Info>(); p.p = dev_params(h->cfg);
  p.cnt = dev_cnt(h); p.work = h->d_work.as<int>(); p.n_work = nw;
  p.draft = h->d_draft.as<uint8_t>(); p.tpos = h->d_tpos.as<int32_t>();
  p.eD = h->s_eD.as<uint8_t>(); p.ecap = ecap;
  p.lw_first = h->s_lw.as<int>(); p.lw_last = p.lw_first + (size_t)NLcap * NWcap * slots_p; p.NLcap = NLcap; p.NWcap = NWcap;
  p.wrec = h->d_wrec.as<WinRec>(); p.wlay = h->d_wlay.as<WLayer>(); p.win_base = h->d_wbase.as<int>();
  p.wcap = (int)std::min<long long>(wcap, 0x7fffffff);
  const int bonus4 = 4 * (h->cfg.pol_match - h->cfg.pol_mismatch);
  p.sub_shift = -1;
  for (int b = 2; b <= 12; ++b) if (bonus4 == 1 << b) p.sub_shift = b;
  if (const char* e = getenv("C3_DEBUG_PREP_ROWS")) p.rows_old = !strcmp(e, "old");
  HIPCHK(zero_counters(h));
  HIPCHK(hipEventRecord(h->ev[5], h->stream));
  DBG("prep: slots=%d ecap=%lld NL=%d NW=%d wcap=%lld\n", slots_p, (long long)ecap, NLcap, NWcap, (long long)wcap);
  c3k_launch_prep(&p, slots_p, h->stream);
  HIPCHK(hipGetLastError());
  HIPCHK(hipEventRecord(h->ev[6], h->stream));
  C3Counters c;
  HIPCHK(read_counters(h, &c));
  h->tm.cells_polish += c.cells; h->tm.cells_polish_computed += c.cells;
  const int n_win = (int)std::min<long long>(c.n_windows, std::min<long long>(wcap, 0x7fffffff));
  h->n_windows = n_win;
  DBG("prep done: n_win=%d\n", n_win);
  const int wout_cap = 3 * WL + 64;
  HIPCHK(hipEventRecord(h->ev[7], h->stream));
  if (n_win > 0) {
    HIPCHK(h->d_wout.ensure((size_t)n_win * wout_cap));
    const int Ncap = 3 * WL + 40 * NLcap, K = NLcap + 2;
    const long long hcap_full = (long long)(Ncap + 1) * 64 * std::max(12, (WL + WL / 2 + 64) / 64);
    const int R_typ = std::min(Ncap, WL + WL / 4 + 30 * NLcap + 64);
    long long hcap = std::min(hcap_full, (long long)(R_typ + R_typ / 2 + 4) * 256);
    if (const char* e = getenv("C3_DEBUG_HCAP_DIV")) hcap = std::max(4096LL, hcap_full / std::max(1, atoi(e)) / 64 * 64);
    const WinLayout L = c3_win_layout(Ncap, K, hcap), L2 = c3_win_layout(Ncap, K, hcap_full);
    const int slots = auto_slots(h, h->cfg.slots_win, L.total, n_win, 20);
    const size_t budget = h->mem_total ? h->mem_total / 3 : ((size_t)64 << 30), per2 = L2.H + L2.D;
    size_t budget2 = budget / 4;
    if (hcap < hcap_full && per2 * 256 > budget2) {
      size_t fr = 0, tot = 0;
      if (hipMemGetInfo(&fr, &tot) == hipSuccess) budget2 = std::min(budget2, fr / 2); else (void)hipGetLastError();
    }
    if (L.total > budget || (hcap < hcap_full && per2 > budget2))
      return c3_fail(h, C3_E_NOMEM, "pol_window: the scratch of one window (DP cells for 3 * pol_window + 40 nodes per layer, 1.5 * pol_window columns) does not fit the device memory set aside for it");
    const int slots2 = hcap < hcap_full ? (int)std::min<size_t>(std::min(slots, 256), budget2 / per2) : 0;
    const size_t S = (size_t)slots, S2 = (size_t)slots2;
    HIPCHK(h->s_win_i.ensure(L.ints * S + 64)); HIPCHK(h->s_win_nk.ensure(L.edges * S));
    HIPCHK(h->s_win_h.ensure(L.H * S)); HIPCHK(h->s_win_d.ensure(L.D * S + 256));
    HIPCHK(h->s_win_b.ensure(L.bases * S)); HIPCHK(h->s_win_sc.ensure(L.score * S)); HIPCHK(h->s_win_desc.ensure(L.desc * S));
    if (slots2) {
      HIPCHK(h->s_win_h2.ensure(L2.H * S2)); HIPCHK(h->s_win_d2.ensure(L2.D * S2 + 256));
      HIPCHK(h->d_wovf.ensure(sizeof(int) * (size_t)n_win));
    }
    WinArgs a; memset(&a, 0, sizeof(a));
    a.b = dev_batch(h); a.p = dev_params(h->cfg); a.cnt = dev_cnt(h); a.n_win = n_win;
    a.wrec_in = h->d_wrec.as<WinRec>(); a.wrec = h->d_wrec.as<WinRec>(); a.wlay = h->d_wlay.as<WLayer>(); a.NLcap = NLcap;
    a.draft = h->d_draft.as<uint8_t>();
    a.ibase = h->s_win_i.as<int>(); a.ebase = h->s_win_nk.as<int>();
    a.base = h->s_win_b.as<uint8_t>(); a.score = h->s_win_sc.as<long long>();
    a.H = h->s_win_h.as<int32_t>(); a.D = h->s_win_d.as<uint16_t>(); a.rdesc = h->s_win_desc.as<uint4>(); a.Ncap = Ncap; a.K = K; a.hcap = hcap; a.Lcap = std::min(std::min(Ncap, 2 * WL + 30 * NLcap), ((getenv("C3_DEBUG_WIN_LDS") ? atoi(getenv("C3_DEBUG_WIN_LDS")) : 6656) - 16) / 6);
    if (const char* e = getenv("C3_DEBUG_WIN_LCAP")) a.Lcap = std::max(64, std::min(Ncap, atoi(e)));
    a.wout = h->d_wout.as<uint8_t>(); a.wout_cap = wout_cap;
    HIPCHK(zero_counters(h));
    if (const char* e = getenv("C3_DEBUG_BAND")) a.band_mode = !strcmp(e, "off") ? 1 : !strcmp(e, "fail") ? 2 : !strcmp(e, "verify") ? 3 : 0;
    if (const char* e = getenv("C3_DEBUG_WIN_CHAIN")) a.no_chain = !strcmp(e, "0");
    a.ovf_list = slots2 ? h->d_wovf.as<int>() : nullptr;
    c3k_launch_window(&a, slots, h->stream);
    HIPCHK(hipGetLastError());
    if (slots2) {
      a.H = h->s_win_h2.as<int32_t>(); a.D = h->s_win_d2.as<uint16_t>(); a.hcap = hcap_full;
      a.wlist = h->d_wovf.as<int>(); a.ovf_list = nullptr;
      c3k_launch_window(&a, slots2, h->stream);
      HIPCHK(hipGetLastError());
    }
    HIPCHK(hipMemcpyAsync(h->phase_win, dev_cnt(h)->phases, sizeof(h->phase_win), hipMemcpyDeviceToHost, h->stream));
  }
  HIPCHK(hipEventRecord(h->ev[8], h->stream));
  StitchArgs s; memset(&s, 0, sizeof(s));
  s.b = dev_batch(h); s.info = h->d_info.as<C3Info>(); s.work = h->d_work.as<int>(); s.n_work = nw;
  s.wrec = h->d_wrec.as<WinRec>(); s.win_base = h->d_wbase.as<int>(); s.wout = h->d_wout.as<uint8_t>(); s.wout_cap = wout_cap;
  s.cons = h->d_cons.as<char>(); s.zflag = h->d_zflag.as<uint8_t>();
  DBG("stitch\n");
  c3k_launch_stitch(&s, std::min(nw, h->n_cus * 16), h->stream);
  HIPCHK(hipGetLastError());
  HIPCHK(hipEventRecord(h->ev[9], h->stream));
  HIPCHK(read_counters(h, &c));
  if (n_win > 0) {
    h->tm.n_win_redo = c.win_ovf; h->tm.cells_polish += c.cells; h->tm.cells_polish_computed += c.cells_computed;
    h->tm.n_band_layers = c.band_layers; h->tm.n_band_fallback = c.band_fallback; h->tm.n_band_mismatch = c.band_mismatch;
    if (c.band_mismatch) fprintf(stderr, "c3poa: band verify mismatch in window %d layer %d (R = %d): last differing base q = %d, band row %d, full row %d, row of q+1 = %d\n",
                                 c.verify.window, c.verify.layer, c.verify.R, c.verify.q, c.verify.band_row, c.verify.full_row, c.verify.next_row);
  }
  HIPCHK(hipEventElapsedTime(ms_prep, h->ev[5], h->ev[6]));
  HIPCHK(hipEventElapsedTime(ms_win, h->ev[7], h->ev[8]));
  HIPCHK(hipEventElapsedTime(ms_st, h->ev[8], h->ev[9]));
  h->tm.n_windows = n_win;
  return 0;
}

static const long long QV_BUDGET = 1LL << 30;
int c3h::qv_scratch(c3_handle* h, long long max_m, long long max_n, int n_items, QvArgs& a, int* grid) {
  a.dir_words = (max_m + 7) / 8 * 64;
  a.lds_n = (int)std::min<long long>((max_n + 15) / 16 * 16, c3k_qv_lds_max());
  a.gcap = max_n > a.lds_n ? (max_n + 15) / 16 * 16 : 0;
  const long long per_wg = 4 * 4 * a.dir_words + 5 * a.gcap;
  *grid = (int)std::max(1LL, std::min<long long>(std::min(n_items, h->n_cus * 8), QV_BUDGET / per_wg));
  HIPCHK(h->s_qv_dirs.ensure(sizeof(uint32_t) * (size_t)a.dir_words * 4 * (size_t)*grid + 256));
  if (a.gcap) HIPCHK(h->s_qv_g.ensure((size_t)a.gcap * 5 * (size_t)*grid + 256));
  a.dirs = h->s_qv_dirs.as<uint32_t>();
  a.gS = a.gcap ? h->s_qv_g.as<int>() : nullptr; a.gcodes = a.gcap ? h->s_qv_g.as<uint8_t>() + (size_t)a.gcap * 4 * (size_t)*grid : nullptr;
  HIPCHK(h->d_qv_cnt.ensure(64));
  HIPCHK(hipMemsetAsync(h->d_qv_cnt.p, 0, 64, h->stream));
  a.cnt = h->d_qv_cnt.as<unsigned long long>();
  return 0;
}
static int qv_counts(c3_handle* h, float ms) {
  unsigned long long c[8];
  HIPCHK(hipMemcpyAsync(c, h->d_qv_cnt.p, 64, hipMemcpyDeviceToHost, h->stream));
  HIPCHK(hipStreamSynchronize(h->stream));
  h->qtm.ms_qv = ms; h->qtm.n_reads = (int64_t)c[0]; h->qtm.n_pieces = (int64_t)c[1]; h->qtm.n_skipped = (int64_t)c[2];
  h->qtm.band_cells = (int64_t)c[3]; h->qtm.edge_hits = (int64_t)c[4];
  return 0;
}

static int run_qv(c3_handle* h) {
  for (int i = 0; i < 2; ++i) if (!h->ev_qv[i]) HIPCHK(hipEventCreate(&h->ev_qv[i]));
  HIPCHK(h->d_qv.ensure((size_t)h->total + 64));
  QvArgs a; memset(&a, 0, sizeof(a));
  int grid = 0;
  int rc = c3h::qv_scratch(h, h->maxL, h->maxL, h->n, a, &grid);
  if (rc) return rc;
  a.n_reads = h->n; a.info = h->d_info.as<C3Info>(); a.pk = h->d_pk.as<uint32_t>(); a.woff = h->d_woff.as<int64_t>();
  a.qual = h->d_qual.as<uint8_t>(); a.off = h->d_off.as<int64_t>(); a.cons = h->d_cons.as<char>(); a.qv = h->d_qv.as<char>();
  a.sa_np = -1;
  DBG("qv: grid=%d dir_words=%lld lds_n=%d gcap=%lld\n", grid, a.dir_words, a.lds_n, a.gcap);
  HIPCHK(hipEventRecord(h->ev_qv[0], h->stream));
  c3k_launch_qv(&a, grid, h->stream);
  HIPCHK(hipGetLastError());
  HIPCHK(hipEventRecord(h->ev_qv[1], h->stream));
  HIPCHK(hipEventSynchronize(h->ev_qv[1]));
  float ms = 0; HIPCHK(hipEventElapsedTime(&ms, h->ev_qv[0], h->ev_qv[1]));
  return qv_counts(h, ms);
}

extern "C" int c3_batch_run(c3_handle* h, int stages) {
  if (!h || h->n <= 0) return C3_E_STATE;
  if ((stages & C3_STAGE_QV) && !((stages | h->stages_done) & C3_STAGE_POLISH))
    return c3_fail(h, C3_E_STATE, "C3_STAGE_QV needs the polish stage (in this call or an earlier one on the resident batch)");
  HIPCHK(hipSetDevice(h->cfg.device));
  int rc;
  float ms;
  hipEvent_t t0 = h->ev[0], t1 = h->ev[1], t2 = h->ev[2], t3 = h->ev[3], t4 = h->ev[4];
  DBG("run: start n=%d\n", h->n);
  const auto wall0 = std::chrono::steady_clock::now();
  const double alloc0 = c3h::g_alloc_ms;
  if (stages & C3_STAGE_CONK) { h->tm.ms_conk = 0; h->tm.cells_conk = 0; }
  if (stages & C3_STAGE_PEAKS) h->tm.ms_peaks = 0;
  if (stages & C3_STAGE_POA) { h->tm.ms_poa = 0; h->tm.cells_poa = 0; }
  if (stages & C3_STAGE_POLISH) { h->tm.ms_prep = h->tm.ms_window = h->tm.ms_stitch = 0; h->tm.cells_polish = 0; h->tm.cells_polish_computed = 0; h->tm.n_band_layers = h->tm.n_band_fallback = h->tm.n_band_mismatch = 0; h->tm.n_windows = 0; h->tm.n_win_redo = 0; }
  HIPCHK(hipEventRecord(t0, h->stream));
  if (stages & C3_STAGE_CONK) { if ((rc = run_conk(h))) return rc; h->tm.cells_conk = 0; for (int i = 0; i < h->n; ++i) h->tm.cells_conk += (h->off[i + 1] - h->off[i]) * (int64_t)h->max_spl; }
  HIPCHK(hipEventRecord(t1, h->stream));
  if (stages & C3_STAGE_PEAKS) { if ((rc = run_peaks(h))) return rc; }
  HIPCHK(hipEventRecord(t2, h->stream));
  float ms_prep = 0, ms_win = 0, ms_st = 0;
  if (stages & (C3_STAGE_POA | C3_STAGE_POLISH)) {
    DBG("run: conk+peaks launched\n");
    if ((rc = fetch_summary(h))) return rc;
    DBG("run: work list ready (%zu reads)\n", h->work.size());
    HIPCHK(hipEventRecord(t3, h->stream));
    if (stages & C3_STAGE_POA) {
      if ((rc = run_poa(h))) return rc;
    }
    HIPCHK(hipEventRecord(t4, h->stream));
    if (stages & C3_STAGE_POA) {
      C3Counters c;
      HIPCHK(read_counters(h, &c));
      if (!h->work.empty()) h->tm.cells_poa = (int64_t)(c.zero_cells + c.cells);
      h->tm.n_poa_redo = h->n_poa_redo; h->tm.n_poa_redo16 = h->n_poa_redo16;
      DBG("run: poa done\n");
      HIPCHK(hipEventElapsedTime(&ms, t3, t4)); h->tm.ms_poa = ms;
    }
    if (stages & C3_STAGE_POLISH) { if ((rc = run_polish(h, &ms_prep, &ms_win, &ms_st))) return rc; }
  }
  if (stages & C3_STAGE_QV) { if ((rc = run_qv(h))) return rc; }
  HIPCHK(hipStreamSynchronize(h->stream));
  DBG("run: done\n");
  HIPCHK(hipGetLastError());
  if (stages & C3_STAGE_CONK) { HIPCHK(hipEventElapsedTime(&ms, t0, t1)); h->tm.ms_conk = ms; }
  if (stages & C3_STAGE_PEAKS) { HIPCHK(hipEventElapsedTime(&ms, t1, t2)); h->tm.ms_peaks = ms; }
  if (stages & C3_STAGE_POLISH) { h->tm.ms_prep = ms_prep; h->tm.ms_window = ms_win; h->tm.ms_stitch = ms_st; }
  h->tm.ms_total = h->tm.ms_conk + h->tm.ms_peaks + h->tm.ms_poa + h->tm.ms_prep + h->tm.ms_window + h->tm.ms_stitch;
  h->tm.ms_wall = std::chrono::duration<float, std::milli>(std::chrono::steady_clock::now() - wall0).count();
  h->tm.ms_alloc = (float)(c3h::g_alloc_ms - alloc0);
  h->tm.ms_host_gap = h->tm.ms_wall - h->tm.ms_total;
  if (stages & C3_STAGES_ALL) h->stages_done &= ~C3_STAGE_QV;
  h->stages_done |= stages;
  return C3_E_OK;
}
```

c3poa_amd/csrc/k_poa.hip:

```cpp
#include "c3_dev.h"
#include "c3_args.h"
#include "c3_launch.h"
#include <type_traits>

#define WSYNC() __syncthreads()
#define EI(v, k) ((size_t)(k) * (size_t)c.Ncap + (size_t)(v))
#define SRC 0
#define SNK 1


struct Ctx {
  int* I; int* E; char* C; uint8_t* B8; long long* score_; uint4* desc_; int* jump_; int* path_;
  int K, n, Ncap, cells_cap;
  int far_shift;
  int osel;
  int rb_span;
  int two_col;
  const uint32_t* pk;
#ifdef C3_DEBUG_PUNT
  unsigned long long* dbg;
#endif
#define CTX_I(name, k) __device__ __forceinline__ int* name() const { return I + (size_t)(k) * Ncap; }
  CTX_I(n_in, 0) CTX_I(n_out, 1) CTX_I(grp, 2) CTX_I(index, 5) CTX_I(gfirst, 6) CTX_I(glast, 7)
  CTX_I(rem, 8) CTX_I(mpl, 9) CTX_I(mpr, 10) CTX_I(rowm, 11)  CTX_I(anchor, 14) CTX_I(col, 15)
  CTX_I(col2t, 16) CTX_I(nxt, 17) CTX_I(foff, 18)
#undef CTX_I
  __device__ __forceinline__ int* order() const { return I + (size_t)(3 + osel) * Ncap; }
  __device__ __forceinline__ int* order2() const { return I + (size_t)(4 - osel) * Ncap; }
  __device__ __forceinline__ int* in_from() const { return E; }
  __device__ __forceinline__ int* out_to() const { return E + (size_t)Ncap * K; }
  __device__ __forceinline__ int* out_w() const { return E + 2 * (size_t)Ncap * K; }
  __device__ __forceinline__ int far_cap() const { return cells_cap >> far_shift; }
  __device__ __forceinline__ int32_t* H() const { return (int32_t*)(C + 2 * (size_t)cells_cap); }
  __device__ __forceinline__ int32_t* E1() const { return (int32_t*)(C + 2 * (size_t)cells_cap + 4 * (size_t)far_cap()); }
  __device__ __forceinline__ int32_t* E2() const { return (int32_t*)(C + 2 * (size_t)cells_cap + 8 * (size_t)far_cap()); }
  __device__ __forceinline__ uint32_t* D() const { return (uint32_t*)(C + 2 * (size_t)cells_cap + 12 * (size_t)far_cap()); }
  __device__ __forceinline__ uint8_t* D8() const { return (uint8_t*)C; }
  __device__ __forceinline__ uint8_t* P8() const { return (uint8_t*)(C + (size_t)cells_cap); }
  __device__ __forceinline__ uint8_t* base() const { return B8; }
  __device__ __forceinline__ uint8_t* rows2() const { return B8 + (size_t)Ncap; }
  __device__ __forceinline__ long long* score() const { return score_; }
  __device__ __forceinline__ uint4* descA() const { return desc_; }
  __device__ __forceinline__ uint4* descB() const { return desc_ + (size_t)Ncap; }
  __device__ __forceinline__ int* jump() const { return jump_; }
  __device__ __forceinline__ int* path() const { return path_; }
};

__device__ __forceinline__ void g_add_edge(Ctx& c, int u, int v, int w) {
  const int K = c.K;
  for (int k = 0; k < c.n_out()[u]; ++k)
    if (c.out_to()[EI(u, k)] == v) { c.out_w()[EI(u, k)] += w; return; }
  int no = c.n_out()[u], ni = c.n_in()[v];
  c.out_to()[EI(u, no)] = v; c.out_w()[EI(u, no)] = w; c.n_out()[u] = no + 1;
  c.in_from()[EI(v, ni)] = u; c.n_in()[v] = ni + 1;
}

#ifndef GU
#define GU 2
#endif
__device__ void g_blocks(Ctx& c, int lane) {
  int gprev = -1;
  for (int i0 = 0; i0 < c.n; i0 += 64 * GU) {
    int v[GU], r[GU];
#pragma unroll
    for (int u = 0; u < GU; ++u) { const int i = i0 + 64 * u + lane; v[u] = i < c.n ? c.order()[i] : -1; }
#pragma unroll
    for (int u = 0; u < GU; ++u) r[u] = v[u] >= 0 ? c.grp()[v[u]] : -2;
#pragma unroll
    for (int u = 0; u < GU; ++u) {
      const int i = i0 + 64 * u + lane;
      const int rp = wave_shr1(r[u], gprev);
      gprev = wave_bcast(r[u], 63);
      if (v[u] >= 0 && r[u] != rp) { c.gfirst()[r[u]] = i; if (i > 0) c.glast()[rp] = i - 1; }
      if (v[u] >= 0 && i + 1 == c.n) c.glast()[r[u]] = i;
    }
  }
  WSYNC();
}

__device__ void g_reorder(Ctx& c, int n_old, int lane, int* lds, int lds_cap) {
  const int n_new = c.n - n_old;
  const bool inl = n_new <= lds_cap;
  if (inl) { for (int k = lane; k < n_new; k += 64) lds[k] = c.anchor()[k]; WSYNC(); }
  for (int i0 = 0; i0 < n_old; i0 += 64 * GU) {
    int v[GU];
#pragma unroll
    for (int u = 0; u < GU; ++u) { const int i = i0 + 64 * u + lane; v[u] = i < n_old ? c.order()[i] : -1; }
#pragma unroll
    for (int u = 0; u < GU; ++u) {
      const int i = i0 + 64 * u + lane;
      if (v[u] < 0) continue;
      int lo = 0, hi = n_new;
      if (inl) { while (lo < hi) { int m = (lo + hi) >> 1; if (lds[m] < i) lo = m + 1; else hi = m; } }
      else { while (lo < hi) { int m = (lo + hi) >> 1; if (c.anchor()[m] < i) lo = m + 1; else hi = m; } }
      c.order2()[i + lo] = v[u]; c.index()[v[u]] = i + lo;
    }
  }
  for (int k = lane; k < n_new; k += 64) { const int pos = (inl ? lds[k] : c.anchor()[k]) + 1 + k; c.order2()[pos] = n_old + k; c.index()[n_old + k] = pos; }
  c.osel ^= 1;
  WSYNC();
  g_blocks(c, lane);
}

__device__ __forceinline__ int32_t rdcell(const Ctx& c, const int32_t* a, int pb, int pe, int po, int j) {
  return (j < pb || j > pe) ? C3_NEG : a[po + (j - pb)];
}

#ifdef C3_PHASE_PROF
#define PHA , unsigned long long& ph_t0_, unsigned long long (&ph_acc_)[16]
#define PHP , ph_t0_, ph_acc_
#else
#define PHA
#define PHP
#endif
#ifndef C3_NEAR
#define C3_NEAR 1
#endif
#define PADL 3
#define PADR 3
#ifndef C3_NARROW_PR
#define C3_NARROW_PR 6
#endif
#define RING_CELLS_N (C3_NARROW_PR * (PADL + 128 + PADR))
#ifndef C3_WIDE_PW
#define C3_WIDE_PW 256
#endif
#define RING_CELLS_W (3 * (PADL + C3_WIDE_PW + PADR))
#define PQW_N 112
#define PQW_W 60
struct PoaLds { unsigned short ring[3 * (RING_CELLS_W > RING_CELLS_N + PQW_N * 2 / 3 + 2 ? RING_CELLS_W : RING_CELLS_N + PQW_N * 2 / 3 + 2)]; int4 meta[6] ; int base8[8] ; unsigned qpk[PQW_W]; };
__shared__ PoaLds L;
static_assert(sizeof(PoaLds) <= 6656, "24 waves per CU need <= 13 LDS granules of 512 bytes per wave");
static_assert(3 * RING_CELLS_N * 2 + PQW_N * 4 <= sizeof(L.ring), "the NARROW query copy must fit behind the NARROW rings");
#define POA_LDS_INTS ((int)(3 * RING_CELLS_N * sizeof(unsigned short) / sizeof(int)))

#define S9(x) ((x) * 512)
#define NEGS (-(1 << 29))
#define NEG2S (-(1 << 30))
#define S3(x) ((x) * 8)
#define BIAS16 32768
#define NEG16 6000
#define NEG2_16 2000
#define FLOOR16 5000
#define ZHI16 12000
#define GLO16 14400
#define ZLO16 13200
#define RB_LO16 (BIAS16 - 400 * 8)
#define RB_HI16 (BIAS16 + 3000 * 8)
#ifdef C3_EXP_ASMNV
#define C3_ASMV
#else
#define C3_ASMV volatile
#endif
__device__ __forceinline__ int maxu16(int a, int b) { int d; asm C3_ASMV("v_max_u16 %0, %1, %2" : "=v"(d) : "v"(a), "v"(b)); return d; }
__device__ __forceinline__ int minu16(int a, int b) { int d; asm C3_ASMV("v_min_u16 %0, %1, %2" : "=v"(d) : "v"(a), "v"(b)); return d; }
__device__ __forceinline__ int cv_16to9(int v, int b8) { return v >= ZLO16 ? (int)((unsigned)(v - BIAS16 + b8) << 6) : NEGS; }
__device__ __forceinline__ int cv_9to16(int x9, int b8, int& bad) {
  if (x9 <= NEGS / 2) return NEG16;
  const int r = (x9 >> 6) - b8 + BIAS16;
  if (r < GLO16 || r > 62000) bad = 1;
  return r;
}


__device__ void poa_sweep_desc(Ctx& c, int lane, int Q, bool qlds, const int PR) {
  const int n = c.n;
  int* hops = c.col();
  for (int c0 = ((n - 1) >> 6) << 6; c0 >= 0; c0 -= 64) {
    const int idx = c0 + lane;
    const bool live = idx < n;
    const int v = live ? c.order()[idx] : SNK;
    const int nin = live ? c.n_in()[v] : 0, nout = live ? c.n_out()[v] : 0;
    int bw = INT32_MIN, bt = SNK;
    unsigned far = 0;
    for (int k = 0; __builtin_amdgcn_ballot_w64(k < nout) != 0; ++k) {
      if (k < nout) {
        const int t = c.out_to()[EI(v, k)], ww = c.out_w()[EI(v, k)];
// ... 651 lines not shown
        const int v = wave_bcast((int)A.x, cl);
        const int cty = wave_bcast(ty, cl);
        const int p0 = wave_bcast((int)B.x, cl), p1 = wave_bcast((int)B.y, cl), p2 = wave_bcast((int)B.z, cl), p3 = wave_bcast((int)B.w, cl);
        unsigned mp, c1, c2, hts, hs, f1x, f2x;
        if (cty == 2 || !wave_bcast((int)hit, cl)) {
          const int cb = wave_bcast(b, cl), cro = wave_bcast(ro, cl);
          if (cty == 2) {
            const unsigned wv = c.D()[c.foff()[i] + (j - cb)];
            mp = wv & 0xff; c1 = (wv >> 8) & 0x1ff; c2 = (wv >> 17) & 0x1ff; hts = (wv >> 26) & 3; hs = (wv >> 28) & 3; f1x = (wv >> 30) & 1; f2x = wv >> 31;
          } else {
            const unsigned db = c.D8()[(unsigned)(cro + (j - cb))];
            const unsigned pb = cty == 1 ? c.P8()[(unsigned)(cro + (j - cb))] : 0u;
            mp = pb & 3; c1 = (((pb >> 2) & 3) << 1) | ((~db) & 1u); c2 = (((pb >> 4) & 3) << 1) | (((~db) >> 1) & 1u);
            hts = 2u - ((db >> 2) & 3u); hs = 2u - ((db >> 4) & 3u); f1x = (db >> 6) & 1; f2x = db >> 7;
          }
        } else {
          const unsigned db = (unsigned)wave_bcast((int)d, cl), pb = (unsigned)wave_bcast((int)pq, cl);
          mp = pb & 3; c1 = (((pb >> 2) & 3) << 1) | ((~db) & 1u); c2 = (((pb >> 4) & 3) << 1) | (((~db) >> 1) & 1u);
          hts = 2u - ((db >> 2) & 3u); hs = 2u - ((db >> 4) & 3u); f1x = (db >> 6) & 1; f2x = db >> 7;
        }
#define TB_PRED(k) ((k) == 0 ? p0 : (k) == 1 ? p1 : (k) == 2 ? p2 : (k) == 3 ? p3 : c.index()[c.in_from()[EI(v, (k))]])
        for (bool same = true; same;) {
          if (st == 0) { st = hs == 0 ? 1 : (hs == 1 ? 4 : 5); }
          else if (st == 1) {
            if (hts == 0) { if (lane == 0) vq[j - 1] = v; const int k = (int)mp; i = TB_PRED(k); --j; st = 0; same = false; }
            else st = hts == 1 ? 2 : 3;
          }
          else if (st == 2) { const int k = (int)(c1 >> 1); i = TB_PRED(k); st = (c1 & 1) ? 2 : 0; same = false; }
          else if (st == 3) { const int k = (int)(c2 >> 1); i = TB_PRED(k); st = (c2 & 1) ? 3 : 0; same = false; }
          else if (st == 4) { if (lane == 0) vq[j - 1] = -1; st = f1x ? 4 : 1; --j; same = false; }
          else { if (lane == 0) vq[j - 1] = -1; st = f2x ? 5 : 1; --j; same = false; }
        }
#undef TB_PRED
        if (i == 0 && j == 0) break;
        if (i < 0 || j < 0) { rc = -2; break; }
        const int drift = (jt - j) - (it - i);
        if (it - i >= 64 || drift > 4 || drift < -20) break;
      }
      WSYNC();
    }
  }
  WSYNC();
  PH_MARK(2)
  return rc;
}
#undef mt9
#undef mm9
#undef e1_9
#undef e2_9
#undef o1_9
#undef o2_9
#undef oe1_9
#undef oe2_9
#undef le1
#undef le2

__device__ int poa_fuse(Ctx& c, bool first, int qb, int Q, int* path, int lane PHA) {
  const int n_old = c.n, K = c.K;
  int* vq = c.mpl();
  if (first) { for (int q = lane; q < Q; q += 64) vq[q] = -1; WSYNC(); }
  int carry_anchor = 0 , carry_new = 0;
  for (int q0 = 0; q0 < Q; q0 += 64) {
    const int q = q0 + lane;
    const bool act = q < Q;
    const int v = act ? vq[q] : -1;
    const int cb = act ? c3_code_at(c.pk, qb + q) : 0;
    int tgt = -1, gnew = -1, anc = -1;
    if (v >= 0) {
      const int rr = c.grp()[v];
      anc = c.glast()[rr];
      if (c.base()[v] == cb) tgt = v;
      else for (int i = c.gfirst()[rr]; i <= anc; ++i) { int x = c.order()[i]; if (c.base()[x] == cb) { tgt = x; break; } }
      if (tgt < 0) gnew = rr;
    }
    const int isnew = act && tgt < 0;
    const int as = max(wave_scan_max(anc), carry_anchor);
    carry_anchor = wave_bcast(as, 63);
    const int ps = wave_scan_add(isnew);
    const int k = carry_new + ps - isnew;
    carry_new += wave_bcast(ps, 63);
    if (isnew) {
      const int id = n_old + k;
      if (id < c.Ncap) { c.base()[id] = (uint8_t)cb; c.n_in()[id] = 0; c.n_out()[id] = 0; c.grp()[id] = gnew >= 0 ? gnew : id; c.anchor()[k] = as; }
      tgt = id;
    }
    if (act) path[q] = tgt;
  }
  const int nn = n_old + carry_new;
  if (nn > c.Ncap) return -1;
  WSYNC();
  for (int q = lane; q <= Q; q += 64) {
    const int u = q == 0 ? SRC : path[q - 1], v = q == Q ? SNK : path[q];
    const int no = c.n_out()[u];
    int hit = -1;
    for (int k = 0; k < no; ++k) if (c.out_to()[EI(u, k)] == v) { hit = k; break; }
    if (hit >= 0) c.out_w()[EI(u, hit)] += 1;
    else {
      const int ni = c.n_in()[v];
      c.out_to()[EI(u, no)] = v; c.out_w()[EI(u, no)] = 1; c.n_out()[u] = no + 1;
      c.in_from()[EI(v, ni)] = u; c.n_in()[v] = ni + 1;
    }
  }
  WSYNC();
  c.n = nn;
  PH_MARK(3)
  g_reorder(c, n_old, lane, (int*)&L.ring[0], POA_LDS_INTS);
  PH_MARK(4)
  return 0;
}

__device__ void normalize_len(const uint8_t* row, int msa_len, const uint8_t* qual, int qlen, uint8_t* out) {
  int si = 0, qi = 0, n = 0;
  while (qi < qlen) {
    if (row[si] != 4) { out[n++] = qual[qi]; ++qi; ++si; }
    else if (qi == 0) { out[n++] = qual[qi]; ++si; }
    else { out[n++] = (uint8_t)(((int)qual[qi - 1] + (int)qual[qi]) / 2); ++si; }
  }
  if (n != msa_len) { int gap = 0; while (gap < msa_len && row[msa_len - 1 - gap] == 4) { out[n] = out[n - 1]; ++n; ++gap; } }
}

__device__ int pairwise_merge(const uint8_t* rowA, const uint8_t* rowB, int ncol, const uint8_t* qa, const uint8_t* qb_,
                              uint8_t* draft, int* col2t) {
  int o = 0, i = 0;
  while (i != ncol) {
    const int A = rowA[i], B = rowB[i];
    if (A == B) { if (A != 4) { if (col2t) col2t[i] = o; draft[o++] = (uint8_t)A; } }
    if (A != B && A != 4 && B != 4) { if (col2t) col2t[i] = o; draft[o++] = (uint8_t)((qa[i] > qb_[i]) ? A : B); }
    if (A == 4 || B == 4) {
      int gl = 1; const uint8_t* gs = (A == 4) ? rowA : rowB;
      for (;;) { if (i + gl >= ncol) { gl = 1; break; } if (gs[i + gl] == 4) ++gl; else break; }
      long sa = 0, sb = 0;
      for (int k = i; k < i + gl && k < ncol; ++k) { sa += qa[k]; sb += qb_[k]; }
      const uint8_t* srcr = (sa > sb) ? rowA : rowB;
      for (int k = i; k < i + gl && k < ncol; ++k) if (srcr[k] != 4) { if (col2t) col2t[k] = o; draft[o++] = srcr[k]; }
      i += gl; continue;
    }
    ++i;
  }
  return o;
}

__global__ void k_pairwise(const uint8_t* rows, int ncol, const uint8_t* qualA, int lenA, const uint8_t* qualB, int lenB,
                           uint8_t* scratch, uint8_t* out, int* out_len) {
  if (threadIdx.x != 0 || blockIdx.x != 0) return;
  normalize_len(rows, ncol, qualA, lenA, scratch);
  normalize_len(rows + ncol, ncol, qualB, lenB, scratch + ncol);
  out_len[0] = pairwise_merge(rows, rows + ncol, ncol, scratch, scratch + ncol, out, nullptr);
}
extern "C" void c3k_launch_pairwise(const uint8_t* rows, int ncol, const uint8_t* qa, int la, const uint8_t* qb, int lb,
                                    uint8_t* scratch, uint8_t* out, int* out_len, hipStream_t s) {
  hipLaunchKernelGGL(k_pairwise, dim3(1), dim3(64), 0, s, rows, ncol, qa, la, qb, lb, scratch, out, out_len);
}

#ifndef C3_POA_WAVES
#define C3_POA_WAVES 6
#endif
template <bool W32, bool DEF, bool WIDE>
__global__ __launch_bounds__(64, C3_POA_WAVES) void k_poa(PoaArgs a) {
  const int lane = wave_lane();
  const int slot = blockIdx.x;
  Ctx c;
  const size_t N = (size_t)a.Ncap;
  c.I = a.ibase + (size_t)slot * C3_POA_NI * N; c.path_ = a.pbase + (size_t)slot * a.Pcap; c.E = a.ebase + (size_t)slot * 3 * N * a.K;
  c.far_shift = c3_poa_far_shift(W32);
  c.C = a.cellsb + (size_t)slot * c3_poa_layout(N, a.K, a.cells_cap, c.far_shift, a.Pcap).cells; c.B8 = a.bbase + (size_t)slot * 5 * N;
  c.score_ = a.score + (size_t)slot * N; c.desc_ = a.desc + (size_t)slot * 2 * N; c.jump_ = a.jump + (size_t)slot * C3_JUMP_LEVELS * N;
  c.K = a.K; c.Ncap = a.Ncap; c.cells_cap = a.cells_cap; c.osel = 0; c.rb_span = a.rb_span > 0 ? a.rb_span : RB_HI16 - RB_LO16; c.two_col = !a.no2col;
#ifdef C3_DEBUG_PUNT
  c.dbg = a.cnt->phases;
#endif
  PH_DECL

  for (;;) {
    int wi = 0;
    if (lane == 0) wi = atomicAdd(&a.cnt->queue, 1);
    wi = wave_first(wi);
    if (wi >= a.n_work) break;
    const int rid = a.work[wi];
    C3Info* info = &a.info[rid];
    const int ns = info->n_sub;
    const int64_t off = a.b.off[rid];
    c.pk = a.b.pk + a.b.woff[rid];
    uint8_t* draft = a.draft + off;
    int32_t* tpos = a.tpos + off;
    const uint8_t* qual = a.b.qual + off;
    long long cells = 0;
    int C = 0, fail = 0; bool punted = false;
    if (ns == 1) {
      const int qb = info->sub_beg[0]; C = info->sub_end[0] - qb;
      for (int k = lane; k < C; k += 64) { draft[k] = (uint8_t)c3_code_at(c.pk, qb + k); tpos[qb + k] = k; }
    } else {
      c.osel = 0;
      if (lane == 0) {
        c.base()[SRC] = 0; c.base()[SNK] = 0; c.n_in()[SRC] = c.n_out()[SRC] = c.n_in()[SNK] = c.n_out()[SNK] = 0;
        c.grp()[SRC] = SRC; c.grp()[SNK] = SNK; c.order()[0] = SRC; c.order()[1] = SNK; c.index()[SRC] = 0; c.index()[SNK] = 1;
      }
      c.n = 2;
      WSYNC();
      g_blocks(c, lane);
      int poff = 0;
      for (int s = 0; s < ns && !fail; ++s) {
        const int qb = wave_first(info->sub_beg[s]), Q = wave_first(info->sub_end[s]) - qb;
        if (s > 0) { const int rc = poa_align<W32, DEF, WIDE>(c, a.p, qb, Q, lane, &cells PHP); if (rc < 0) { fail = (rc == -4 || rc == -5) ? 2 : 1; punted = rc == -5; break; } }
        if (poa_fuse(c, s == 0, qb, Q, c.path() + poff, lane PHP) < 0) { fail = 2; break; }
        poff += Q;
      }
      PH_MARK(9)
      if (!fail) {
        int ncol_acc = 0;
        for (int i0 = 0; i0 < c.n; i0 += 64) {
          const int i = i0 + lane;
          int v = -1, start = 0;
          if (i < c.n) {
            v = c.order()[i];
            if (v != SRC && v != SNK) start = (i == 0) || (c.grp()[v] != c.grp()[c.order()[i - 1]]) || c.order()[i - 1] == SRC;
          }
          const int ps = wave_scan_add(start);
          if (i < c.n) c.col()[v] = (v == SRC || v == SNK) ? -1 : ncol_acc + ps - 1;
          ncol_acc += wave_bcast(ps, 63);
        }
        WSYNC();
        PH_MARK(5)
        const int ncol = ncol_acc;
        for (int i = lane; i < ncol; i += 64) c.col2t()[i] = -1;
        if (a.msa_dbg) {
          uint8_t* dbg = a.msa_dbg + a.msa_off[rid];
          for (int i = lane; i < ns * ncol; i += 64) dbg[i] = 4;
          WSYNC();
          int po = 0;
          for (int s = 0; s < ns; ++s) {
            const int Q = info->sub_end[s] - info->sub_beg[s];
            for (int k = lane; k < Q; k += 64) { int v = c.path()[po + k]; dbg[(size_t)s * ncol + c.col()[v]] = c.base()[v]; }
            po += Q;
          }
          if (lane == 0) a.msa_len[rid] = ncol;
        }
        WSYNC();
        if (ns == 2) {
          uint8_t* rowA = c.rows2(); uint8_t* rowB = c.rows2() + ncol;
          uint8_t* qa = c.rows2() + 2 * (size_t)ncol; uint8_t* qb_ = c.rows2() + 3 * (size_t)ncol;
          for (int i = lane; i < 2 * ncol; i += 64) c.rows2()[i] = 4;
          WSYNC();
          const int b0 = info->sub_beg[0], l0 = info->sub_end[0] - b0, b1 = info->sub_beg[1], l1 = info->sub_end[1] - b1;
          for (int k = lane; k < l0; k += 64) { int v = c.path()[k]; rowA[c.col()[v]] = c.base()[v]; }
          for (int k = lane; k < l1; k += 64) { int v = c.path()[l0 + k]; rowB[c.col()[v]] = c.base()[v]; }
          WSYNC();
          if (lane == 0) {
            bool same = (l0 == l1);
            for (int k = 0; same && k < l0; ++k) same = c3_code_at(c.pk, b0 + k) == c3_code_at(c.pk, b1 + k);
            normalize_len(rowA, ncol, same ? qual + b1 : qual + b0, l0, qa);
            normalize_len(rowB, ncol, qual + b1, l1, qb_);
            const int o = pairwise_merge(rowA, rowB, ncol, qa, qb_, draft, c.col2t());
            c.rem()[0] = o;
          }
          WSYNC();
          C = c.rem()[0];
        } else {
          {
            const int n = c.n;
            int* scp = c.jump(); int* hpp = c.jump() + (size_t)c.Ncap; int* nxp = c.jump() + 2 * (size_t)c.Ncap;
            int* onf = c.jump() + 3 * (size_t)c.Ncap;
            for (int c0 = ((n - 1) >> 6) << 6; c0 >= 0; c0 -= 64) {
              const int idx = c0 + lane;
              const bool live = idx < n;
              const int v = live ? c.order()[idx] : SNK;
              const int no = (live && v != SNK) ? c.n_out()[v] : 0;
              int bw = INT32_MIN, bt = SNK, cm = 0;
              for (int k = 0; __builtin_amdgcn_ballot_w64(k < no) != 0; ++k) {
                if (k < no) {
                  const int ww = c.out_w()[EI(v, k)];
                  if (ww > bw) { bw = ww; bt = c.out_to()[EI(v, k)]; cm = 1; } else if (ww == bw) ++cm;
                }
              }
              bool tie = cm >= 2;
              int acc = no > 0 ? bw : (v == SNK ? 0 : INT32_MIN / 2), hp = no > 0 ? 1 : 0;
              int ptr = (no > 0 && !tie) ? c.index()[bt] : -1;
              int np = ptr;
              bool done = no == 0;
              if (ptr >= c0 + 64) { acc += scp[ptr]; hp += hpp[ptr]; ptr = -1; done = true; }
              for (;;) {
                for (int r = 0; r < 6 && __builtin_amdgcn_ballot_w64(!done && !tie) != 0; ++r) {
                  const int src = (max(ptr, c0) - c0) << 2;
                  const int a2 = __builtin_amdgcn_ds_bpermute(src, acc), h2 = __builtin_amdgcn_ds_bpermute(src, hp);
                  const int p2 = __builtin_amdgcn_ds_bpermute(src, ptr);
                  const int d2 = __builtin_amdgcn_ds_bpermute(src, (int)done), t2 = __builtin_amdgcn_ds_bpermute(src, (int)tie);
                  if (!done && !tie && ptr >= 0) {
                    if (d2) { acc += a2; hp += h2; ptr = -1; done = true; }
                    else if (!t2) { acc += a2; hp += h2; ptr = p2; }
                  }
                }
                const unsigned long long tm = __builtin_amdgcn_ballot_w64(tie && !done);
                if (!tm) break;
                const int T = 63 - __builtin_clzll(tm);
                const int vT = __builtin_amdgcn_readlane(v, T), noT = __builtin_amdgcn_readlane(no, T);
                int tbw = INT32_MIN, tbt = SNK, tsb = 0, thp = 0, tnp = -1;
                for (int k = 0; k < noT; ++k) {
                  const int wk = c.out_w()[EI(vT, k)], tk = c.out_to()[EI(vT, k)];
                  const int pk_ = c.index()[tk];
                  int sk, hk;
                  if (pk_ >= c0 + 64) { sk = scp[pk_]; hk = hpp[pk_]; }
                  else { sk = wave_bcast(acc, pk_ - c0); hk = wave_bcast(hp, pk_ - c0); }
                  if (wk > tbw) { tbw = wk; tbt = tk; tsb = sk; thp = hk; tnp = pk_; }
                  else if (wk == tbw && tsb <= sk) { tbt = tk; tsb = sk; thp = hk; tnp = pk_; }
                }
                if (lane == T) { acc = tbw + tsb; hp = 1 + thp; np = tnp; done = true; tie = false; ptr = -1; }
              }
              if (live) { scp[idx] = acc; hpp[idx] = hp; nxp[idx] = np; onf[idx] = 0; }
              WSYNC();
            }
            unsigned* const Lf = (unsigned*)&L.ring[0];
            C = hpp[0] - 1;
            if (lane == 0) onf[0] = 1;
            WSYNC();
            for (int c0 = 0; c0 < n && C > 0; c0 += 64) {
              const int idx = c0 + lane;
              const bool live = idx < n;
              int on = live ? onf[idx] : 0;
              const int np = live ? nxp[idx] : -1;
              int J = (np >= c0 && np < c0 + 64) ? np - c0 : -1;
              for (int r = 0; r < 6; ++r) {
                Lf[lane] = 0;
                WSYNC();
                if (on && J >= 0) Lf[J] = 1;
                WSYNC();
                on |= (int)Lf[lane];
                const int J2 = __builtin_amdgcn_ds_bpermute(max(J, 0) << 2, J);
                J = J >= 0 ? J2 : -1;
                WSYNC();
              }
              if (on && np >= c0 + 64) onf[np] = 1;
              if (on && live) {
                const int v = c.order()[idx];
                if (v != SRC && v != SNK) { const int pp = C - hpp[idx]; draft[pp] = c.base()[v]; c.col2t()[c.col()[v]] = pp; }
              }
              WSYNC();
            }
            if (C < 0) C = 0;
            WSYNC();
          }

        }
        PH_MARK(6)
        int poff2 = 0;
        for (int s = 0; s < ns; ++s) {
          const int qb = info->sub_beg[s], Q = info->sub_end[s] - qb;
          for (int k = lane; k < Q; k += 64) tpos[qb + k] = c.col2t()[c.col()[c.path()[poff2 + k]]];
          poff2 += Q;
        }
      }
    }
    WSYNC();
    PH_MARK(7)
    const bool to16 = punted || a.overflow == nullptr;
    int* const olist = to16 ? a.overflow16 : a.overflow;
    const bool redo = fail == 2 && olist != nullptr;
    if (lane == 0) {
      if (redo) olist[atomicAdd(to16 ? &a.cnt->poa_ovf16 : &a.cnt->poa_ovf, 1)] = rid;
      else {
        info->draft_len = C;
        if (fail) { info->status = C3_ST_LIMIT; info->draft_len = 0; }
        else if (C == 0) info->status = C3_ST_NO_CONSENSUS;
        atomicAdd(&a.cnt->cells, (unsigned long long)cells);
      }
    }
    WSYNC();
  }
  PH_FLUSH(a.cnt->phases)
}

extern "C" void c3k_launch_poa(const PoaArgs* a, int slots, int wide32, int wide_ring, hipStream_t stream) {
  const C3Params& p = a->p;
  const bool def = p.poa_match == 5 && p.poa_mismatch == 4 && p.o1 == 4 && p.e1 == 2 && p.o2 == 24 && p.e2 == 1;
#define C3_POA_LAUNCH(W, D, R) hipLaunchKernelGGL((k_poa<W, D, R>), dim3(slots), dim3(64), 0, stream, *a)
  if (wide32) { if (def) C3_POA_LAUNCH(true, true, false); else C3_POA_LAUNCH(true, false, false); }
  else if (wide_ring) { if (def) C3_POA_LAUNCH(false, true, true); else C3_POA_LAUNCH(false, false, true); }
  else { if (def) C3_POA_LAUNCH(false, true, false); else C3_POA_LAUNCH(false, false, false); }
#undef C3_POA_LAUNCH
}
```

include/c3poa.h:

```cpp
#ifndef C3POA_H
#define C3POA_H
#include <stdint.h>

#ifdef __cplusplus
extern "C" {
#endif

#define C3_MAX_PEAKS 256

typedef enum {
  C3_E_OK = 0,
  C3_E_NO_DEVICE = -1,
  C3_E_HIP = -2,
  C3_E_ARG = -3,
  C3_E_NOMEM = -4,
  C3_E_STATE = -5,
  C3_E_LIMIT = -6,
  C3_E_DATA = -7
} c3_err;

typedef enum {
  C3_ST_OK = 0,
  C3_ST_NOT_ASSIGNED = 1,
  C3_ST_NO_PEAKS = 2,
  C3_ST_NO_CONSENSUS = 3,
  C3_ST_TOO_SHORT = 4,
  C3_ST_LIMIT = 5
} c3_status;

typedef struct {
  int device;
  int conk_match, conk_mismatch, conk_penalty;
  int sg_iters, sg_window, sg_order;
  int mdistcutoff;
  int poa_match, poa_mismatch;
  int poa_o1, poa_e1, poa_o2, poa_e2;
  int poa_band_b; double poa_band_f;
  int pol_match, pol_mismatch, pol_gap;
  int pol_window, pol_q;
  int dang_band;
  int slots_poa, slots_win;
  int zero;
  int64_t zero_max_cells;
} c3_config;

typedef struct {
  int32_t status;
  int32_t n_peaks;
  int32_t n_sub;
  int32_t has_front, has_tail;
  int32_t front_end, tail_beg;
  int32_t cons_len, draft_len;
  int32_t n_win;
  int32_t peaks[C3_MAX_PEAKS];
  int32_t sub_beg[C3_MAX_PEAKS], sub_end[C3_MAX_PEAKS];
} c3_read_result;

typedef struct {
  float ms_pack, ms_conk, ms_peaks, ms_poa, ms_prep, ms_window, ms_stitch, ms_total;
  int64_t n_reads, n_bases, n_windows;
  int64_t cells_conk, cells_poa, cells_polish;
  int64_t n_poa_redo;
  float ms_wall;
  float ms_host_worklist;
  float ms_alloc;
  float ms_host_gap;
  int64_t cells_polish_computed;
  int64_t n_band_layers, n_band_fallback;
  int64_t n_band_mismatch;
  int64_t n_win_redo;
  int64_t n_poa_redo16;
} c3_timing;

typedef struct c3_handle c3_handle;

void c3_default_config(c3_config* cfg);
const char* c3_version(void);
int c3_device_count(void);
int c3_warm_device(int device);

int c3_create(const c3_config* cfg, c3_handle** out);
void c3_destroy(c3_handle* h);
const char* c3_last_error(const c3_handle* h);

int c3_set_splints(c3_handle* h, int n, const char* cat, const int64_t* off);

int c3_batch_upload(c3_handle* h, int n, const char* seqs, const char* quals, const int64_t* off,
                    const int16_t* splint_id, const char* strand);

int c3_batch_stage(c3_handle* h, int n, const char* seqs, const char* quals, const int64_t* off,
                   const int16_t* splint_id, const char* strand);
int c3_batch_commit(c3_handle* h);

int c3_batch_assign(c3_handle* h, const int16_t* splint_id, const char* strand);

#define C3_STAGE_CONK 1
#define C3_STAGE_PEAKS 2
#define C3_STAGE_POA 4
#define C3_STAGE_POLISH 8
#define C3_STAGES_ALL 15
int c3_batch_run(c3_handle* h, int stages);
int c3_batch_sync(c3_handle* h);

int c3_batch_results(c3_handle* h, c3_read_result* res, char* cons, int64_t cons_cap, int64_t* cons_off);
int c3_batch_results_snapshot(c3_handle* h);
int c3_batch_results_fetch(c3_handle* h, c3_read_result* res, char* cons, int64_t cons_cap, int64_t* cons_off);
int c3_batch_timing(c3_handle* h, c3_timing* t);

int c3_fetch_track(c3_handle* h, int read, int32_t* out, int64_t cap);
int c3_fetch_smoothed(c3_handle* h, int read, double* out, int64_t cap);
int c3_fetch_raw_peaks(c3_handle* h, int read, int32_t* out, int cap);
int c3_fetch_draft(c3_handle* h, int read, char* out, int cap);
int c3_fetch_msa2(c3_handle* h, int read, char* rowA, char* rowB, int cap);

int c3_call_peaks(c3_handle* h, const int32_t* scores, int n, int min_dist, int32_t* peaks, int cap, double* smoothed);
int c3_poa_msa(c3_handle* h, int n, const char* const* seqs, const int* lens,
               char* cons, int cons_cap, int* cons_len, char* msa, int64_t msa_cap, int* msa_len);
int c3_pairwise_consensus(c3_handle* h, const char* rowA, const char* rowB, int msa_len,
                          const char* subA, int lenA, const char* qualA, const char* subB, int lenB, const char* qualB,
                          char* out, int cap, int* out_len);
int c3_determine_consensus(c3_handle* h, int n, const char* const* subs, const char* const* quals,
                           const int* lens, const char* front, const char* front_q, int front_len,
                           const char* tail, const char* tail_q, int tail_len,
                           char* out, int cap, int* out_len, char* draft, int draft_cap, int* draft_len);

int c3_scan_splints(c3_handle* h, int32_t* out, int16_t* assign_splint, char* assign_strand);

int c3_scan_adapters(c3_handle* h, int32_t* out);

int c3_zero_repeats(c3_handle* h, const char* d0, const char* q0, int n0, const char* d1, const char* q1, int n1,
                    int min_len, char* out, int cap, int* out_len);


typedef struct {
  int32_t n;
  int64_t n_short;
  const char* names;
  const int64_t* name_off;
  const char* seqs;
  const char* quals;
  const int64_t* off;
} c3_host_batch;

int c3_host_alloc(int64_t bytes, void** out);
void c3_host_free(void* p);

typedef struct c3_reader c3_reader;
int c3_reader_open(const char* path, int n_sets, c3_reader** out);
int c3_reader_open_range(const char* path, int n_sets, int64_t beg, int64_t end, c3_reader** out);
void c3_reader_close(c3_reader* r);
const char* c3_reader_error(const c3_reader* r);
int64_t c3_reader_noqual(const c3_reader* r);
int64_t c3_reader_reserved_bytes(const c3_reader* r);
int c3_reader_range_lost(const c3_reader* r);
void c3_reader_names_only(c3_reader* r, int names_only);
int c3_reader_next(c3_reader* r, int max_reads, int64_t max_bases, int min_len, c3_host_batch* out);
int c3_reader_next_set(c3_reader* r, int set, int max_reads, int64_t max_bases, int min_len, c3_host_batch* out);

int c3_write_group(const c3_host_batch* b, const c3_read_result* res, const char* cons, const int64_t* cons_off,
                   const int16_t* splint_id, int n_splints, const char* const* cons_paths,
                   const char* const* sub_paths, int zero);

void c3_writer_reset(void);

typedef struct c3_assign c3_assign;
int c3_assign_open(const char* psl_path, int n_splints, const char* const* splint_names, c3_assign** out);
void c3_assign_close(c3_assign* a);
int c3_assign_batch(const c3_assign* a, const c3_host_batch* b, int16_t* splint_id, char* strand);
int c3_assign_seen(const c3_assign* a, uint8_t* flags, int64_t* rows_kept);

int c3_write_splint_psl(const c3_host_batch* b, const int32_t* table, const int16_t* splint_id, const char* strand,
                        int n_splints, const char* const* splint_names, const int32_t* splint_lens, int match,
                        const char* path, int64_t* rows_written);

int c3_match_index_batch(c3_handle* h, int n, const char* pieces, const int32_t* lens, int n_idx,
                         const char* idx_cat, const int64_t* idx_off, int32_t* out);

int c3_match_index(const char* seq, int n, int n_idx, const char* idx_cat, const int64_t* idx_off);

#define C3_DEMUX_HEAD 300
#define C3_DEMUX_MAX_IDX 128
#define C3_DEMUX_MAX_LEN 32
#define C3_DEMUX_MAX_BYTES 31
int c3_demux_indexes(c3_handle* h, int n, const char* heads, int n_a, const char* a_cat, const int64_t* a_off,
                     int n_b, const char* b_cat, const int64_t* b_off, int32_t* win, uint8_t* dist);
int c3_demux_host(int n, const char* heads, int n_a, const char* a_cat, const int64_t* a_off,
                  int n_b, const char* b_cat, const int64_t* b_off, int32_t* win, uint8_t* dist);

#define C3_STAGE_QV 16
#define C3_QV_BAND 128
#define C3_QV_MAX 60
#define C3_QV_MATCH 2
#define C3_QV_MISMATCH (-4)
#define C3_QV_GAP (-4)
#define C3_QV_SKEW 4
#define C3_QV_MAX_PIECES 252
#define C3_QV_GLOBAL 0
#define C3_QV_ANCHOR_START 1
#define C3_QV_ANCHOR_END 2

typedef struct {
  float ms_qv;
  int64_t n_reads;
  int64_t n_pieces;
  int64_t n_skipped;
  int64_t band_cells;
  int64_t edge_hits;
} c3_qv_timing;
int c3_batch_qv_timing(c3_handle* h, c3_qv_timing* t);

int c3_batch_results_fetch_qv(c3_handle* h, c3_read_result* res, char* cons, int64_t cons_cap, int64_t* cons_off, char* qv);
int c3_batch_results_qv(c3_handle* h, c3_read_result* res, char* cons, int64_t cons_cap, int64_t* cons_off, char* qv);

int c3_consensus_qv(c3_handle* h, const char* cons, int n, int n_pieces, const char* seq_cat, const char* qual_cat,
                    const int64_t* piece_off, const int32_t* modes, char* qv_out);
int c3_consensus_qv_host(const char* cons, int n, int n_pieces, const char* seq_cat, const char* qual_cat,
                         const int64_t* piece_off, const int32_t* modes, char* qv_out);

int c3_write_consensus_fastq(const c3_host_batch* b, const c3_read_result* res, const char* cons, const int64_t* cons_off,
                             const char* qv, const int16_t* splint_id, int n_splints, const char* const* fq_paths, int zero);

typedef struct c3_bgzf c3_bgzf;
int c3_bgzf_create(int device, c3_bgzf** out);
void c3_bgzf_destroy(c3_bgzf* z);
// ... 137 lines not shown
```

Baseline: 424,900.

## Precompute second-subread POA alignment with a specialised banded pairwise kernel

Adds a k_poa_pair kernel that runs before the main POA pass. It aligns the second subread to the first as a plain sequence-to-sequence banded alignment using 16-bit biased scores and register/LDS rings, then records the traceback as a per-base vertex map. The main POA kernel checks a done flag and reuses that map for subread 1 instead of running the general graph alignment, which is meant to cut the cost of the first graph alignment per read. This adds an extra launch and traceback storage, declines reads that fall outside its band limits, and runs serially before the main kernel on the same stream.

```diff
diff --git a/c3poa_amd/_lib.py b/c3poa_amd/_lib.py
--- a/c3poa_amd/_lib.py
+++ b/c3poa_amd/_lib.py
@@ -66,7 +66,8 @@
                                          "ms_stitch", "ms_total")] + \
                [(n, C.c_int64) for n in ("n_reads", "n_bases", "n_windows", "cells_conk", "cells_poa", "cells_polish", "n_poa_redo")] + \
                [(n, C.c_float) for n in ("ms_wall", "ms_host_worklist", "ms_alloc", "ms_host_gap")] + \
-               [(n, C.c_int64) for n in ("cells_polish_computed", "n_band_layers", "n_band_fallback", "n_band_mismatch", "n_win_redo", "n_poa_redo16")]
+               [(n, C.c_int64) for n in ("cells_polish_computed", "n_band_layers", "n_band_fallback", "n_band_mismatch", "n_win_redo", "n_poa_redo16", "n_pair", "n_pair_declined")] + \
+               [("ms_poa_pair", C.c_float)]
 
 
 def _fields_dict(t):
diff --git a/c3poa_amd/csrc/c3_args.h b/c3poa_amd/csrc/c3_args.h
--- a/c3poa_amd/csrc/c3_args.h
+++ b/c3poa_amd/csrc/c3_args.h
@@ -10,6 +10,8 @@
   unsigned long long zero_cells;
   int poa_ovf;
   int poa_ovf16;
+  int pair_queue;
+  int n_pair, n_pair_declined;
   int n_windows;
   int win_ovf;
   int win_queue2;
@@ -42,8 +44,21 @@
   int* pbase;
   int* overflow;
   int* overflow16;
+  const uint8_t* pair_done; const uint16_t* pair_vq; const int* pair_cells;
+};
+struct PoaPairArgs {
+  C3Batch b; const C3Info* info; C3Params p; C3Counters* cnt; const int* work; int n_work;
+  int* ibase; char* cellsb;
+  size_t dstride; int dbytes;
+  int Ncap, cells_cap, rb_span;
+  uint16_t* vq;
+  int* cells; uint8_t* done;
 };
 #define C3_POA_NI 19
+#define C3_POA_I_ROWM 11
+__host__ __device__ inline bool c3_poa_default_scoring(const C3Params& p) {
+  return p.poa_match == 5 && p.poa_mismatch == 4 && p.o1 == 4 && p.e1 == 2 && p.o2 == 24 && p.e2 == 1;
+}
 __host__ __device__ inline int c3_poa_far_shift(bool w32) { return w32 ? 0 : 2; }
 struct PoaLayout { size_t ints, edges, cells, bases, score, desc, jump, path, total; };
 __host__ __device__ inline PoaLayout c3_poa_layout(size_t Ncap, size_t K, int cells_cap, int far_shift, size_t Pcap) {
diff --git a/c3poa_amd/csrc/c3_handle.hip b/c3poa_amd/csrc/c3_handle.hip
--- a/c3poa_amd/csrc/c3_handle.hip
+++ b/c3poa_amd/csrc/c3_handle.hip
@@ -196,7 +196,7 @@
   (void)hipSetDevice(h->cfg.device);
   for (hipStream_t s : {h->stream, h->stream_up, h->stream_dn}) if (s) (void)hipStreamSynchronize(s);
   for (hipStream_t s : {h->stream, h->stream_up, h->stream_dn}) if (s) (void)hipStreamDestroy(s);
-  for (hipEvent_t ev : {h->ev_dn, h->ev_up[0], h->ev_up[1], h->ev_qv[0], h->ev_qv[1]}) if (ev) (void)hipEventDestroy(ev);
+  for (hipEvent_t ev : {h->ev_dn, h->ev_up[0], h->ev_up[1], h->ev_qv[0], h->ev_qv[1], h->ev_pair[0], h->ev_pair[1]}) if (ev) (void)hipEventDestroy(ev);
   for (hipEvent_t ev : h->ev) if (ev) (void)hipEventDestroy(ev);
   for (hipEvent_t ev : h->ev_post) if (ev) (void)hipEventDestroy(ev);
   for (hipEvent_t ev : h->ev_fa) if (ev) (void)hipEventDestroy(ev);
diff --git a/c3poa_amd/csrc/c3_host.h b/c3poa_amd/csrc/c3_host.h
--- a/c3poa_amd/csrc/c3_host.h
+++ b/c3poa_amd/csrc/c3_host.h
@@ -137,6 +137,7 @@
   DBuf s_poa_i, s_poa_nk, s_poa_cells, s_poa_b, s_poa_sc, s_poa_desc, s_poa_jump, s_poa_path, d_overflow;
   int n_poa_redo = 0;
   int n_poa_redo16 = 0;
+  DBuf d_pair_vq, d_pair_cells, d_pair_done; hipEvent_t ev_pair[2] = {nullptr, nullptr}; bool pair_ran = false; int n_pair = 0, n_pair_declined = 0;
   DBuf s_eD, s_lw, d_wrec, d_wlay, d_wbase, d_wout;
   DBuf s_win_i, s_win_nk, s_win_h, s_win_d, s_win_b, s_win_sc, s_win_desc, s_win_h2, s_win_d2, d_wovf;
   DBuf s_zero_d, d_zinfo, d_zflag, d_zwork; std::vector<int> zwork;
diff --git a/c3poa_amd/csrc/c3_launch.h b/c3poa_amd/csrc/c3_launch.h
--- a/c3poa_amd/csrc/c3_launch.h
+++ b/c3poa_amd/csrc/c3_launch.h
@@ -3,7 +3,7 @@
 #include <stddef.h>
 #include <stdint.h>
 
-struct ConkArgs; struct AdapterArgs; struct PostArgs; struct PeaksArgs; struct PoaArgs; struct PrepArgs; struct WinArgs; struct StitchArgs;
+struct ConkArgs; struct AdapterArgs; struct PostArgs; struct PeaksArgs; struct PoaArgs; struct PoaPairArgs; struct PrepArgs; struct WinArgs; struct StitchArgs;
 struct ZeroArgs; struct QvArgs; struct C3BgzfMember; struct C3FqHdr; struct C3BamHdr; struct C3BamTile; struct FaArgs; struct EmitArgs; struct FxArgs; struct DsArgs;
 
 extern "C" {
@@ -12,6 +12,7 @@
 void c3k_launch_match_index(const char*, const int*, int, int, const char*, const long long*, int*, hipStream_t);
 void c3k_launch_pairwise(const uint8_t*, int, const uint8_t*, int, const uint8_t*, int, uint8_t*, uint8_t*, int*, hipStream_t);
 void c3k_launch_poa(const PoaArgs*, int, int, int, hipStream_t);
+void c3k_launch_poa_pair(const PoaPairArgs*, int, hipStream_t);
 void c3k_launch_post_classify(const PostArgs*, hipStream_t);
 void c3k_launch_post_scan(const PostArgs*, hipStream_t);
 void c3k_launch_post_emit(const PostArgs*, hipStream_t);
diff --git a/c3poa_amd/csrc/c3_stages.hip b/c3poa_amd/csrc/c3_stages.hip
--- a/c3poa_amd/csrc/c3_stages.hip
+++ b/c3poa_amd/csrc/c3_stages.hip
@@ -182,7 +182,7 @@
   return 0;
 }
 
-static int launch_poa(c3_handle* h, const int* d_work, int nw, int Ncap, int K, int Pcap, long long cells, int* d_overflow, int* d_overflow16, int waves_per_cu, int wide_ring) {
+static int launch_poa(c3_handle* h, const int* d_work, int nw, int Ncap, int K, int Pcap, long long cells, int* d_overflow, int* d_overflow16, int waves_per_cu, int wide_ring, bool first_pass = false) {
   cells = (cells + 15) & ~15LL;
   cells = (cells + 63) & ~63LL;
   const bool w32 = d_overflow16 == nullptr || getenv("C3_DEBUG_POA32");
@@ -205,6 +205,25 @@
   a.msa_dbg = nullptr; a.msa_off = nullptr; a.msa_len = nullptr;
   if (h->debug_msa) { a.msa_dbg = h->d_msa.as<uint8_t>(); a.msa_off = h->d_msa_off.as<int64_t>(); a.msa_len = h->d_msa_len.as<int>(); }
   DBG("poa: nw=%d Ncap=%d K=%d cells=%lld slots=%d (%.1f MB per slot)%s\n", nw, Ncap, K, cells, slots, L.total / 1048576.0, d_overflow ? "" : (d_overflow16 ? " [full-size pass]" : " [32-bit pass]"));
+  const bool def = c3_poa_default_scoring(a.p);
+  const char* pe = getenv("C3_DEBUG_POA_PAIR");
+  if (first_pass && def && !w32 && !wide_ring && !(pe && atoi(pe) == 0)) {
+    HIPCHK(h->d_pair_vq.ensure(sizeof(uint16_t) * (size_t)h->total + 64)); HIPCHK(h->d_pair_cells.ensure(sizeof(int) * (size_t)h->n));
+    HIPCHK(h->d_pair_done.ensure((size_t)h->n));
+    for (int i = 0; i < 2; ++i) if (!h->ev_pair[i]) HIPCHK(hipEventCreate(&h->ev_pair[i]));
+    HIPCHK(hipMemsetAsync(h->d_pair_done.p, 0, (size_t)h->n, h->stream));
+    PoaPairArgs q; memset(&q, 0, sizeof(q));
+    q.b = a.b; q.info = a.info; q.p = a.p; q.cnt = a.cnt; q.work = d_work; q.n_work = nw;
+    q.ibase = a.ibase; q.cellsb = a.cellsb; q.dstride = L.cells; q.dbytes = (int)std::min<size_t>(L.cells, (size_t)1 << 30);
+    q.Ncap = Ncap; q.cells_cap = (int)cells; q.rb_span = a.rb_span;
+    q.vq = h->d_pair_vq.as<uint16_t>(); q.cells = h->d_pair_cells.as<int>(); q.done = h->d_pair_done.as<uint8_t>();
+    HIPCHK(hipEventRecord(h->ev_pair[0], h->stream));
+    c3k_launch_poa_pair(&q, slots, h->stream);
+    HIPCHK(hipGetLastError());
+    HIPCHK(hipEventRecord(h->ev_pair[1], h->stream));
+    a.pair_done = q.done; a.pair_vq = q.vq; a.pair_cells = q.cells;
+    h->pair_ran = true;
+  }
   c3k_launch_poa(&a, slots, w32 ? 1 : 0, wide_ring, h->stream);
   HIPCHK(hipGetLastError());
   return 0;
@@ -239,14 +258,17 @@
   C3Counters* dc = dev_cnt(h);
   HIPCHK(zero_cnt(h, &dc->queue)); HIPCHK(zero_cnt(h, &dc->cells)); HIPCHK(zero_cnt(h, &dc->poa_ovf)); HIPCHK(zero_cnt(h, &dc->poa_ovf16));
   HIPCHK(zero_cnt(h, &dc->phases));
+  HIPCHK(zero_cnt(h, &dc->pair_queue)); HIPCHK(zero_cnt(h, &dc->n_pair)); HIPCHK(zero_cnt(h, &dc->n_pair_declined));
+  h->pair_ran = false; h->n_pair = 0; h->n_pair_declined = 0;
   int wide_ring = (max_q > 1792 || 2 * w + 1 + 24 > 128) ? 1 : 0;
   if (const char* e_ = getenv("C3_DEBUG_POA_WIDE")) wide_ring = atoi(e_) ? 1 : 0;
   int* ovA = h->d_overflow.as<int>(); int* ovB = h->d_overflow.as<int>() + nw;
-  int rc = launch_poa(h, h->d_work.as<int>(), nw, Ncap, K, Pcap, cells, ovA, ovB, 24, wide_ring);
+  int rc = launch_poa(h, h->d_work.as<int>(), nw, Ncap, K, Pcap, cells, ovA, ovB, 24, wide_ring, true);
   if (rc) return rc;
   h->n_poa_redo = 0; h->n_poa_redo16 = 0;
   C3Counters c;
   HIPCHK(read_counters(h, &c));
+  h->n_pair = c.n_pair; h->n_pair_declined = c.n_pair_declined;
   if (c.poa_ovf > 0) {
     h->n_poa_redo = c.poa_ovf;
     HIPCHK(zero_cnt(h, &dc->queue));
@@ -449,7 +471,7 @@
   const double alloc0 = c3h::g_alloc_ms;
   if (stages & C3_STAGE_CONK) { h->tm.ms_conk = 0; h->tm.cells_conk = 0; }
   if (stages & C3_STAGE_PEAKS) h->tm.ms_peaks = 0;
-  if (stages & C3_STAGE_POA) { h->tm.ms_poa = 0; h->tm.cells_poa = 0; }
+  if (stages & C3_STAGE_POA) { h->tm.ms_poa = 0; h->tm.cells_poa = 0; h->tm.ms_poa_pair = 0; h->tm.n_pair = h->tm.n_pair_declined = 0; h->pair_ran = false; h->n_pair = h->n_pair_declined = 0; }
   if (stages & C3_STAGE_POLISH) { h->tm.ms_prep = h->tm.ms_window = h->tm.ms_stitch = 0; h->tm.cells_polish = 0; h->tm.cells_polish_computed = 0; h->tm.n_band_layers = h->tm.n_band_fallback = h->tm.n_band_mismatch = 0; h->tm.n_windows = 0; h->tm.n_win_redo = 0; }
   HIPCHK(hipEventRecord(t0, h->stream));
   if (stages & C3_STAGE_CONK) { if ((rc = run_conk(h))) return rc; h->tm.cells_conk = 0; for (int i = 0; i < h->n; ++i) h->tm.cells_conk += (h->off[i + 1] - h->off[i]) * (int64_t)h->max_spl; }
@@ -471,6 +493,8 @@
       HIPCHK(read_counters(h, &c));
       if (!h->work.empty()) h->tm.cells_poa = (int64_t)(c.zero_cells + c.cells);
       h->tm.n_poa_redo = h->n_poa_redo; h->tm.n_poa_redo16 = h->n_poa_redo16;
+      h->tm.n_pair = h->n_pair; h->tm.n_pair_declined = h->n_pair_declined;
+      if (h->pair_ran) { HIPCHK(hipEventElapsedTime(&ms, h->ev_pair[0], h->ev_pair[1])); h->tm.ms_poa_pair = ms; }
       DBG("run: poa done\n");
       HIPCHK(hipEventElapsedTime(&ms, t3, t4)); h->tm.ms_poa = ms;
     }
diff --git a/c3poa_amd/csrc/k_poa.hip b/c3poa_amd/csrc/k_poa.hip
--- a/c3poa_amd/csrc/k_poa.hip
+++ b/c3poa_amd/csrc/k_poa.hip
@@ -22,7 +22,7 @@
 #endif
 #define CTX_I(name, k) __device__ __forceinline__ int* name() const { return I + (size_t)(k) * Ncap; }
   CTX_I(n_in, 0) CTX_I(n_out, 1) CTX_I(grp, 2) CTX_I(index, 5) CTX_I(gfirst, 6) CTX_I(glast, 7)
-  CTX_I(rem, 8) CTX_I(mpl, 9) CTX_I(mpr, 10) CTX_I(rowm, 11)  CTX_I(anchor, 14) CTX_I(col, 15)
+  CTX_I(rem, 8) CTX_I(mpl, 9) CTX_I(mpr, 10) CTX_I(rowm, C3_POA_I_ROWM)  CTX_I(anchor, 14) CTX_I(col, 15)
   CTX_I(col2t, 16) CTX_I(nxt, 17) CTX_I(foff, 18)
 #undef CTX_I
   __device__ __forceinline__ int* order() const { return I + (size_t)(3 + osel) * Ncap; }
@@ -980,6 +980,11 @@
   hipLaunchKernelGGL(k_pairwise, dim3(1), dim3(64), 0, s, rows, ncol, qa, la, qb, lb, scratch, out, out_len);
 }
 
+__device__ __attribute__((noinline)) void pair_fetch(int* vq, const uint16_t* pv, int Q) {
+  for (int k = wave_lane(); k < Q; k += 64) { const int v = pv[k]; vq[k] = v == 0xffff ? -1 : v; }
+  WSYNC();
+}
+
 #ifndef C3_POA_WAVES
 #define C3_POA_WAVES 6
 #endif
@@ -1029,7 +1034,11 @@
       int poff = 0;
       for (int s = 0; s < ns && !fail; ++s) {
         const int qb = wave_first(info->sub_beg[s]), Q = wave_first(info->sub_end[s]) - qb;
-        if (s > 0) { const int rc = poa_align<W32, DEF, WIDE>(c, a.p, qb, Q, lane, &cells PHP); if (rc < 0) { fail = (rc == -4 || rc == -5) ? 2 : 1; punted = rc == -5; break; } }
+        if (!W32 && DEF && !WIDE && s == 1 && a.pair_done != nullptr && wave_first((int)a.pair_done[rid]) != 0) {
+          pair_fetch(c.mpl(), a.pair_vq + a.b.off[rid] + qb, Q);
+          cells += wave_first(a.pair_cells[rid]);
+        }
+        else if (s > 0) { const int rc = poa_align<W32, DEF, WIDE>(c, a.p, qb, Q, lane, &cells PHP); if (rc < 0) { fail = (rc == -4 || rc == -5) ? 2 : 1; punted = rc == -5; break; } }
         if (poa_fuse(c, s == 0, qb, Q, c.path() + poff, lane PHP) < 0) { fail = 2; break; }
         poff += Q;
       }
@@ -1198,7 +1207,7 @@
 
 extern "C" void c3k_launch_poa(const PoaArgs* a, int slots, int wide32, int wide_ring, hipStream_t stream) {
   const C3Params& p = a->p;
-  const bool def = p.poa_match == 5 && p.poa_mismatch == 4 && p.o1 == 4 && p.e1 == 2 && p.o2 == 24 && p.e2 == 1;
+  const bool def = c3_poa_default_scoring(p);
 #define C3_POA_LAUNCH(W, D, R) hipLaunchKernelGGL((k_poa<W, D, R>), dim3(slots), dim3(64), 0, stream, *a)
   if (wide32) { if (def) C3_POA_LAUNCH(true, true, false); else C3_POA_LAUNCH(true, false, false); }
   else if (wide_ring) { if (def) C3_POA_LAUNCH(false, true, true); else C3_POA_LAUNCH(false, false, true); }
diff --git a/c3poa_amd/csrc/k_poa_pair.hip b/c3poa_amd/csrc/k_poa_pair.hip
--- /dev/null
+++ b/c3poa_amd/csrc/k_poa_pair.hip
@@ -0,0 +1,293 @@
+#include "c3_dev.h"
+#include "c3_args.h"
+#include "c3_launch.h"
+
+#define WSYNC() __syncthreads()
+#define PADL 3
+#define PW 128
+#define PWT (PADL + PW + 3)
+#define PQW 112
+#define DSTRIDE 128
+#define S3(x) ((x) * 8)
+#define BIAS16 32768
+#define NEG16 6000
+#define NEG2_16 2000
+#define FLOOR16 5000
+#define ZHI16 12000
+#define GLO16 14400
+#define ZLO16 13200
+#define RB_LO16 (BIAS16 - 400 * 8)
+#define RB_HI16 (BIAS16 + 3000 * 8)
+__device__ __forceinline__ int maxu16(int a, int b) { int d; asm volatile("v_max_u16 %0, %1, %2" : "=v"(d) : "v"(a), "v"(b)); return d; }
+__device__ __forceinline__ int minu16(int a, int b) { int d; asm volatile("v_min_u16 %0, %1, %2" : "=v"(d) : "v"(a), "v"(b)); return d; }
+
+struct alignas(16) PairLds { union { unsigned short ring[3][2][PWT]; uint8_t win[64 * 32]; }; unsigned qpk[PQW]; };
+__shared__ PairLds L;
+
+__device__ int pair_align(const PoaPairArgs& a, const uint32_t* pk, int qb0, int Q0, int qb1, int Q1, uint8_t* D, int* rowrec, uint16_t* vq, int lane) {
+  constexpr int mt8 = S3(5), mm8 = S3(-4), e1_8 = S3(2), e2_8 = S3(1), o1_8 = S3(4), o2_8 = S3(24), oe1_8 = o1_8 + e1_8, oe2_8 = o2_8 + e2_8;
+  if (Q0 < 1 || Q1 < 1 || Q1 > PQW * 16 || Q0 + 1 >= 0xffff || Q0 + 2 > a.Ncap || (long long)(Q0 + 1) * DSTRIDE + 64 > a.dbytes) return -1;
+  const int rb_span = a.rb_span > 0 ? a.rb_span : RB_HI16 - RB_LO16;
+  const int w = wave_first(a.p.band_b + (int)(a.p.band_f * (double)Q1));
+  const int le1_8 = e1_8 * lane, le2_8 = e2_8 * lane, lo1_8 = le1_8 + o1_8, lo2_8 = le2_8 + o2_8, lane4 = lane * 4;
+  unsigned short (*LH)[PWT] = L.ring[0]; unsigned short (*LE1)[PWT] = L.ring[1]; unsigned short (*LE2)[PWT] = L.ring[2];
+  WSYNC();
+  for (int i = lane; i < PQW && 16 * i < Q1; i += 64) {
+    const long long b0 = (long long)qb1 + 16 * i;
+    const unsigned w0 = pk[b0 >> 4], w1 = pk[(b0 >> 4) + 1];
+    L.qpk[i] = __builtin_amdgcn_alignbit(w1, w0, (unsigned)(b0 & 15) * 2);
+  }
+  { unsigned* r32 = (unsigned*)&L.ring[0][0][0]; for (int i = lane; i < 3 * 2 * PWT / 2; i += 64) r32[i] = NEG16 | (NEG16 << 16); }
+  WSYNC();
+  int u_beg = 0, u_end = min(Q1, max(Q1 - Q0, 0) + w), u_left = 0, u_right = 0, u_b8 = 0;
+  if (u_end + 1 > PW) return -1;
+  int ncell = u_end + 1;
+  int pH = NEG16, pE1 = NEG16, pE2 = NEG16;
+#pragma unroll
+  for (int ch = 0; ch < 2; ++ch) {
+    const int j = 64 * ch + lane;
+    const int sc = j == 0 ? 0 : max(-(4 + 2 * j), -(24 + j));
+    const int h = j <= u_end ? BIAS16 + S3(sc) : NEG16;
+    const unsigned d = j == 0 ? 40u : (8u | ((j <= 20 ? 1u : 0u) << 4) | (j >= 2 ? 192u : 0u));
+    LH[0][PADL + j] = (unsigned short)h;
+    if (j <= u_end) D[j] = (uint8_t)d;
+    if (ch == 0) pH = h;
+  }
+  bool pv_ok = u_end + 1 <= 64;
+  bool in_ring = true; int rs = 0;
+  int gacc = 0xffff, punt = 0;
+  for (int ib = 0; ib <= Q0; ib += 64) {
+    const int ridx = ib + lane;
+    const int vbv = (ridx >= 1 && ridx <= Q0) ? c3_code_at(pk, (int64_t)qb0 + ridx - 1) : 0;
+    int recv = (ib == 0 && lane == 0) ? ((u_end + 1) << 16) : 0;
+    const int cnt = min(64, Q0 + 1 - ib);
+    for (int li = ib == 0 ? 1 : 0; li < cnt; ++li) {
+      const int idx = ib + li;
+      const int qr = Q1 - Q0 + idx;
+      const int vb = __builtin_amdgcn_readlane(vbv, li);
+      const bool nonempty = u_end >= u_beg;
+      const int mplv = nonempty ? u_left + 1 : INT32_MAX / 2, mprv = nonempty ? u_right + 1 : 0;
+      const int beg = max(max(0, min(mplv, qr) - w), u_beg);
+      int end = min(min(Q1, max(mprv, qr) + w), u_end + 1);
+      end = max(end, beg - 1);
+      const int wd = end - beg + 1, sh = beg - u_beg;
+      if (wd < 1 || wd > PW || ncell + PW > a.cells_cap) return -1;
+      uint8_t* const Dr = D + (size_t)idx * DSTRIDE;
+      int left, right, nb8 = u_b8;
+      if (wd <= 64) {
+        const int j = beg + lane;
+        const bool act = lane < wd;
+        const int jq = max(j - 1, 0);
+        const unsigned qw_ = L.qpk[min(jq >> 4, PQW - 1)];
+        int hd, hp, e1p, e2p;
+        if (pv_ok && wd + sh <= 64 && (sh >= 1 || u_end - u_beg < 63)) {
+          const int a_p = lane4 + sh * 4, a_d = a_p - 4;
+          hd = __builtin_amdgcn_ds_bpermute(a_d, pH); hp = __builtin_amdgcn_ds_bpermute(a_p, pH);
+          e1p = __builtin_amdgcn_ds_bpermute(a_p, pE1); e2p = __builtin_amdgcn_ds_bpermute(a_p, pE2);
+        } else {
+          if (!in_ring) {
+            rs ^= 1;
+            LH[rs][PADL + lane] = (unsigned short)pH; LE1[rs][PADL + lane] = (unsigned short)pE1; LE2[rs][PADL + lane] = (unsigned short)pE2;
+            LH[rs][PADL + 64 + lane] = NEG16; LE1[rs][PADL + 64 + lane] = NEG16; LE2[rs][PADL + 64 + lane] = NEG16;
+          }
+          const int ix = PADL + min(max(sh + lane, -2), PW + 1);
+          hd = LH[rs][ix - 1]; hp = LH[rs][ix]; e1p = LE1[rs][ix]; e2p = LE2[rs][ix];
+        }
+        const int qc = (int)((qw_ >> ((jq & 15) * 2)) & 3);
+        const int M = hd + ((vb == qc) ? mt8 + 2 : mm8 + 2);
+        const int E1t = maxu16(hp - (oe1_8 - 1), e1p - e1_8);
+        const int E2t = maxu16(hp - (oe2_8 - 2), e2p - e2_8);
+        const int E1c = E1t & ~7, E2c = E2t & ~7;
+        const int k2 = maxu16(maxu16(M, E1c + 1), E2c);
+        const int ht = k2 & ~7;
+        const int htm = act ? ht : NEG2_16;
+        int s1 = htm + le1_8, s2 = htm + le2_8, s3 = htm;
+        wave_scan_max3(s1, s2, s3);
+        const int px1 = wave_shr1(s1, NEG2_16), px2 = wave_shr1(s2, NEG2_16);
+        const int htl = wave_shr1(htm, NEG16);
+        const int f1 = px1 - lo1_8, f2 = px2 - lo2_8;
+        const int k3 = maxu16(maxu16(ht + 2, f1 + 1), f2);
+        const int h = k3 & ~7;
+        unsigned d = ((unsigned)E1t & 1u) | ((unsigned)E2t & 2u) | (((unsigned)k2 & 3u) << 2) | (((unsigned)k3 & 3u) << 4);
+        d |= (((unsigned)(htl - oe1_8 - f1)) >> 25) & 64u;
+        d |= (((unsigned)(htl - oe2_8 - f2)) >> 24) & 128u;
+        const int rb = __builtin_amdgcn_readlane(s3, 63);
+        const unsigned long long mxm = __ballot(htm == rb);
+        left = beg + __builtin_ctzll(mxm); right = beg + (63 - __builtin_clzll(mxm));
+        pH = maxu16(act ? h : NEG16, FLOOR16); pE1 = act ? E1c : NEG16; pE2 = act ? E2c : NEG16;
+        if ((unsigned)(rb - RB_LO16) > (unsigned)rb_span) {
+          const int m1 = rb - BIAS16, fl1 = FLOOR16 + max(m1, 0);
+          nb8 += m1; punt |= (int)(rb < GLO16);
+          pH = act ? maxu16(h, fl1) - m1 : NEG16; pE1 = act ? maxu16(E1c, fl1) - m1 : NEG16; pE2 = act ? maxu16(E2c, fl1) - m1 : NEG16;
+        }
+        gacc = minu16(gacc, pH - (ZHI16 + 1));
+        Dr[lane] = (uint8_t)d;
+        pv_ok = true; in_ring = false;
+      } else {
+        if (!in_ring) {
+          rs ^= 1;
+          LH[rs][PADL + lane] = (unsigned short)pH; LE1[rs][PADL + lane] = (unsigned short)pE1; LE2[rs][PADL + lane] = (unsigned short)pE2;
+          LH[rs][PADL + 64 + lane] = NEG16; LE1[rs][PADL + 64 + lane] = NEG16; LE2[rs][PADL + 64 + lane] = NEG16;
+        }
+        const int c0l = 2 * lane;
+        const bool act0 = c0l < wd, act1 = c0l + 1 < wd;
+        const int j0 = beg + c0l;
+        const int jq0 = max(j0 - 1, 0), jq1 = j0;
+        const unsigned qw0 = L.qpk[min(jq0 >> 4, PQW - 1)], qw1 = L.qpk[min(jq1 >> 4, PQW - 1)];
+        const int rx = PADL + min(sh + c0l, PW);
+        const int hd0 = LH[rs][rx - 1], hp0 = LH[rs][rx], hp1 = LH[rs][rx + 1];
+        const int e1p0 = LE1[rs][rx], e1p1 = LE1[rs][rx + 1], e2p0 = LE2[rs][rx], e2p1 = LE2[rs][rx + 1];
+        const int qc0 = (int)((qw0 >> ((jq0 & 15) * 2)) & 3), qc1 = (int)((qw1 >> ((jq1 & 15) * 2)) & 3);
+        const int M0 = hd0 + ((vb == qc0) ? mt8 + 2 : mm8 + 2), M1 = hp0 + ((vb == qc1) ? mt8 + 2 : mm8 + 2);
+        const int E1t0 = maxu16(hp0 - (oe1_8 - 1), e1p0 - e1_8), E1t1 = maxu16(hp1 - (oe1_8 - 1), e1p1 - e1_8);
+        const int E2t0 = maxu16(hp0 - (oe2_8 - 2), e2p0 - e2_8), E2t1 = maxu16(hp1 - (oe2_8 - 2), e2p1 - e2_8);
+        const int E1c0 = E1t0 & ~7, E2c0 = E2t0 & ~7, E1c1 = E1t1 & ~7, E2c1 = E2t1 & ~7;
+        const int k20 = maxu16(maxu16(M0, E1c0 + 1), E2c0), k21 = maxu16(maxu16(M1, E1c1 + 1), E2c1);
+        const int ht0 = k20 & ~7, ht1 = k21 & ~7;
+        const int htm0 = act0 ? ht0 : NEG2_16, htm1 = act1 ? ht1 : NEG2_16;
+        const int l1 = e1_8 * c0l, l2 = e2_8 * c0l;
+        const int t10 = htm0 + l1, t20 = htm0 + l2;
+        int s1 = max(t10, htm1 + l1 + e1_8), s2 = max(t20, htm1 + l2 + e2_8), s3 = max(htm0, htm1);
+        wave_scan_max3(s1, s2, s3);
+        const int px1 = wave_shr1(s1, NEG2_16), px2 = wave_shr1(s2, NEG2_16);
+        const int f10 = px1 - o1_8 - l1, f20 = px2 - o2_8 - l2;
+        const int f11 = max(px1, t10) - (o1_8 + e1_8) - l1, f21 = max(px2, t20) - (o2_8 + e2_8) - l2;
+        const int htl0 = wave_shr1(htm1, NEG16);
+        const int k30 = maxu16(maxu16(ht0 + 2, f10 + 1), f20), k31 = maxu16(maxu16(ht1 + 2, f11 + 1), f21);
+        const int h0 = k30 & ~7, h1 = k31 & ~7;
+        unsigned d0 = ((unsigned)E1t0 & 1u) | ((unsigned)E2t0 & 2u) | (((unsigned)k20 & 3u) << 2) | (((unsigned)k30 & 3u) << 4);
+        unsigned d1 = ((unsigned)E1t1 & 1u) | ((unsigned)E2t1 & 2u) | (((unsigned)k21 & 3u) << 2) | (((unsigned)k31 & 3u) << 4);
+        d0 |= (((unsigned)(htl0 - oe1_8 - f10)) >> 25) & 64u; d0 |= (((unsigned)(htl0 - oe2_8 - f20)) >> 24) & 128u;
+        d1 |= (((unsigned)(htm0 - oe1_8 - f11)) >> 25) & 64u; d1 |= (((unsigned)(htm0 - oe2_8 - f21)) >> 24) & 128u;
+        const int rb = __builtin_amdgcn_readlane(s3, 63);
+        const unsigned long long mx0 = __ballot(htm0 == rb), mx1 = __ballot(htm1 == rb);
+        left = beg + min(mx0 ? 2 * (int)__builtin_ctzll(mx0) : 256, mx1 ? 2 * (int)__builtin_ctzll(mx1) + 1 : 256);
+        right = beg + max(mx0 ? 2 * (63 - (int)__builtin_clzll(mx0)) : -1, mx1 ? 2 * (63 - (int)__builtin_clzll(mx1)) + 1 : -1);
+        int vH0 = maxu16(act0 ? h0 : NEG16, FLOOR16), vE10 = act0 ? E1c0 : NEG16, vE20 = act0 ? E2c0 : NEG16;
+        int vH1 = maxu16(act1 ? h1 : NEG16, FLOOR16), vE11 = act1 ? E1c1 : NEG16, vE21 = act1 ? E2c1 : NEG16;
+        if ((unsigned)(rb - RB_LO16) > (unsigned)rb_span) {
+          const int m1 = rb - BIAS16, fl1 = FLOOR16 + max(m1, 0);
+          nb8 += m1; punt |= (int)(rb < GLO16);
+          vH0 = act0 ? maxu16(h0, fl1) - m1 : NEG16; vE10 = act0 ? maxu16(E1c0, fl1) - m1 : NEG16; vE20 = act0 ? maxu16(E2c0, fl1) - m1 : NEG16;
+          vH1 = act1 ? maxu16(h1, fl1) - m1 : NEG16; vE11 = act1 ? maxu16(E1c1, fl1) - m1 : NEG16; vE21 = act1 ? maxu16(E2c1, fl1) - m1 : NEG16;
+        }
+        gacc = minu16(minu16(gacc, vH0 - (ZHI16 + 1)), vH1 - (ZHI16 + 1));
+        *(unsigned short*)(Dr + c0l) = (unsigned short)((d0 & 0xffu) | ((d1 & 0xffu) << 8));
+        rs ^= 1;
+        { const int cb = PADL + c0l;
+          LH[rs][cb] = (unsigned short)vH0; LE1[rs][cb] = (unsigned short)vE10; LE2[rs][cb] = (unsigned short)vE20;
+          LH[rs][cb + 1] = (unsigned short)vH1; LE1[rs][cb + 1] = (unsigned short)vE11; LE2[rs][cb + 1] = (unsigned short)vE21; }
+        pv_ok = false; in_ring = true;
+      }
+      recv = lane == li ? (beg | (wd << 16)) : recv;
+      u_beg = beg; u_end = end; u_left = left; u_right = right; u_b8 = nb8; ncell += wd;
+    }
+    if (lane < cnt) rowrec[ib + lane] = recv;
+  }
+  if (punt != 0 || __builtin_amdgcn_ballot_w64((unsigned)(gacc & 0xffff) < (unsigned)(GLO16 - ZHI16 - 1)) != 0) return -1;
+  {
+    if (Q1 < u_beg || Q1 > u_end) return -1;
+    int hq;
+    if (pv_ok) hq = __builtin_amdgcn_readlane(pH, Q1 - u_beg);
+    else hq = wave_first((int)LH[rs][PADL + Q1 - u_beg]);
+    if (hq < ZLO16) return -1;
+  }
+  WSYNC();
+  int rc = 0;
+  {
+    uint8_t* const WD = &L.win[0];
+    int i = Q0, j = Q1, st = 0;
+    while (!(i == 0 && j == 0) && rc == 0) {
+      const int it = i, jt = j;
+      const int rk = it - lane;
+      const int ic = max(rk, 0);
+      const int rec = rowrec[ic];
+      const int b = rec & 0xffff, e = b + (rec >> 16) - 1, ro = ic * DSTRIDE;
+      int a0 = ro + (jt - lane - 8 - b);
+      a0 = min(max(a0, 0), (int)a.dbytes - 32) & ~3;
+      const int w0 = a0 - ro + b;
+      {
+        const uint32_t* src = (const uint32_t*)(D + a0);
+        const uint4 x0 = make_uint4(src[0], src[1], src[2], src[3]), x1 = make_uint4(src[4], src[5], src[6], src[7]);
+        uint4* wd_ = (uint4*)(WD + lane * 32); wd_[0] = x0; wd_[1] = x1;
+      }
+      WSYNC();
+      for (;;) {
+        const int s = it - i;
+        const int jk = j - (lane - s);
+        const bool inb = rk >= 0 && lane >= s && jk >= b && jk <= e;
+        const int wo = jk - w0;
+        const bool hit = inb && wo >= 0 && wo < 32;
+        const unsigned d = WD[lane * 32 + min(max(wo, 0), 31)];
+        if (st == 0 && i > 0 && j > 0) {
+          const bool ok = hit && rk >= 1 && jk >= 1 && ((d >> 2) & 15u) == 10u;
+          const unsigned long long bal = __ballot(ok) >> s;
+          int m = (~bal) ? __builtin_ctzll(~bal) : 64;
+          m = min(m, 64 - s);
+          if (lane >= s && lane < s + m) vq[jk - 1] = (uint16_t)(rk + 1);
+          i -= m; j -= m;
+          if (i == 0 && j == 0) break;
+          if (s + m >= 64) break;
+        }
+        const int cl = it - i;
+        if (!wave_bcast((int)inb, cl)) { rc = -2; break; }
+        unsigned db;
+        if (wave_bcast((int)hit, cl)) db = (unsigned)wave_bcast((int)d, cl);
+        else db = D[(size_t)i * DSTRIDE + (j - wave_bcast(b, cl))];
+        const unsigned c1 = (~db) & 1u, c2 = ((~db) >> 1) & 1u, hts = 2u - ((db >> 2) & 3u), hs = 2u - ((db >> 4) & 3u), f1x = (db >> 6) & 1u, f2x = db >> 7;
+        for (bool same = true; same;) {
+          if (st == 0) { st = hs == 0 ? 1 : (hs == 1 ? 4 : 5); }
+          else if (st == 1) {
+            if (hts == 0) { if (j < 1) { rc = -2; break; } if (lane == 0) vq[j - 1] = (uint16_t)(i + 1); --i; --j; st = 0; same = false; }
+            else st = hts == 1 ? 2 : 3;
+          }
+          else if (st == 2) { --i; st = c1 ? 2 : 0; same = false; }
+          else if (st == 3) { --i; st = c2 ? 3 : 0; same = false; }
+          else { if (j < 1) { rc = -2; break; } if (lane == 0) vq[j - 1] = 0xffff; st = st == 4 ? (f1x ? 4 : 1) : (f2x ? 5 : 1); --j; same = false; }
+        }
+        if (rc < 0) break;
+        if (i == 0 && j == 0) break;
+        if (i < 0 || j < 0) { rc = -2; break; }
+        const int drift = (jt - j) - (it - i);
+        if (it - i >= 64 || drift > 4 || drift < -20) break;
+      }
+      WSYNC();
+    }
+  }
+  return rc < 0 ? -1 : ncell;
+}
+
+#ifndef C3_PAIR_WAVES
+#define C3_PAIR_WAVES 6
+#endif
+__global__ __launch_bounds__(64, C3_PAIR_WAVES) void k_poa_pair(PoaPairArgs a) {
+  const int lane = wave_lane();
+  const int slot = blockIdx.x;
+  uint8_t* const D = (uint8_t*)a.cellsb + (size_t)slot * (size_t)a.dstride;
+  int* const rowrec = a.ibase + (size_t)slot * C3_POA_NI * (size_t)a.Ncap + C3_POA_I_ROWM * (size_t)a.Ncap;
+  for (;;) {
+    int wi = 0;
+    if (lane == 0) wi = atomicAdd(&a.cnt->pair_queue, 1);
+    wi = wave_first(wi);
+    if (wi >= a.n_work) break;
+    const int rid = a.work[wi];
+    const C3Info* info = &a.info[rid];
+    const int ns = wave_first(info->n_sub);
+    int cells = -1;
+    if (ns >= 2) {
+      const int qb0 = wave_first(info->sub_beg[0]), Q0 = wave_first(info->sub_end[0]) - qb0;
+      const int qb1 = wave_first(info->sub_beg[1]), Q1 = wave_first(info->sub_end[1]) - qb1;
+      cells = pair_align(a, a.b.pk + a.b.woff[rid], qb0, Q0, qb1, Q1, D, rowrec, a.vq + a.b.off[rid] + qb1, lane);
+    }
+    WSYNC();
+    if (lane == 0 && ns >= 2) {
+      if (cells > 0) { a.cells[rid] = cells; a.done[rid] = 1; atomicAdd(&a.cnt->n_pair, 1); }
+      else atomicAdd(&a.cnt->n_pair_declined, 1);
+    }
+    WSYNC();
+  }
+}
+
+extern "C" void c3k_launch_poa_pair(const PoaPairArgs* a, int slots, hipStream_t stream) {
+  hipLaunchKernelGGL(k_poa_pair, dim3(slots), dim3(64), 0, stream, *a);
+}
diff --git a/include/c3poa.h b/include/c3poa.h
--- a/include/c3poa.h
+++ b/include/c3poa.h
@@ -70,6 +70,8 @@
   int64_t n_band_mismatch;
   int64_t n_win_redo;
   int64_t n_poa_redo16;
+  int64_t n_pair, n_pair_declined;
+  float ms_poa_pair;
 } c3_timing;
 
 typedef struct c3_handle c3_handle;
```

Result: faster. 432,400 (median of 6 runs) (+1.8%).
